# ThomasK33/kube-scheduler-simulator

Hardware: AMD Instinct MI355X
Metric: pod x node filter+score evals/sec (higher is better)
Workload: dtype int64

## Files before the change

### include/ksim_engine.h

```cpp
#ifndef KSIM_ENGINE_H
#define KSIM_ENGINE_H

#include <stdint.h>
#include <stddef.h>

#ifdef __cplusplus
extern "C" {
#endif

#define KSIM_ABI_VERSION 12

#define KSIM_KEY_NODE_MASK    ((1 << 18) - 1)
#define KSIM_MAX_NODES        KSIM_KEY_NODE_MASK
#define KSIM_MAX_NODE_TAINTS  8
#define KSIM_TAINT_WORDS      4
#define KSIM_MAX_SCALAR       8
#define KSIM_MAX_LABEL_COLS   256
#define KSIM_EXPR_VALS        6
#define KSIM_MAX_FILTER       16
#define KSIM_MAX_SCORE        8
#define KSIM_MAX_RES          4
#define KSIM_MAX_SHAPE        16
#define KSIM_MAX_USES         16
#define KSIM_MAX_CLASSES      4096
// ... 264 lines not shown
  int32_t n_feasible;
  int32_t n_evaluated;
  int32_t n_processed;
  int32_t k_to_find;
  int32_t next_start;
  int32_t _pad;
} ksim_eval_out;

typedef struct ksim_batch_stats {
  int64_t pods;
  int64_t scheduled;
  int64_t unschedulable;
  int64_t evals;
  double  device_ms;
  int64_t batches;
  int64_t truncations;
  int64_t perpod_cycles;
} ksim_batch_stats;

typedef struct ksim_handle ksim_handle;

int  ksim_abi_version(void);
size_t ksim_abi_sizeof(int which);
int  ksim_create(int device, ksim_handle** out);
void ksim_destroy(ksim_handle* h);
const char* ksim_last_error(const ksim_handle* h);

int ksim_set_profile(ksim_handle* h, const ksim_profile* p);
int ksim_set_cluster(ksim_handle* h, const ksim_node_table* nodes, const ksim_vocab* vocab);
int ksim_upsert_nodes(ksim_handle* h, const ksim_node_table* nodes, const ksim_vocab* vocab, const int32_t* old_pos);
int ksim_remove_node(ksim_handle* h, int32_t pos);
int ksim_update_node_rows(ksim_handle* h, const ksim_node_table* nodes, const ksim_vocab* vocab, const int32_t* rows,
                          int32_t n_rows);
int ksim_get_node_state(ksim_handle* h, int64_t* req_cpu, int64_t* req_mem, int64_t* req_eph,
                        int64_t* nz_cpu, int64_t* nz_mem, int32_t* num_pods);
int ksim_get_nb_alloc(ksim_handle* h, int64_t* out);
int ksim_get_class_count(ksim_handle* h, int32_t* out);
int ksim_get_next_start(ksim_handle* h, int32_t* next_start);
int ksim_set_next_start(ksim_handle* h, int32_t next_start);
int ksim_set_pod_seq(ksim_handle* h, int64_t seq);

int ksim_eval_pod(ksim_handle* h, const ksim_pod_set* pods, int32_t pod_index, ksim_eval_out* out);

int ksim_eval_pod_filter(ksim_handle* h, const ksim_pod_set* pods, int32_t pod_index, ksim_eval_out* out);
int ksim_eval_pod_finish(ksim_handle* h, const uint8_t* ext_fail, const int64_t* ext_score, ksim_eval_out* out);
int ksim_assume(ksim_handle* h, const ksim_pod_set* pods, int32_t pod_index, int32_t node);
int ksim_forget(ksim_handle* h, const ksim_pod_set* pods, int32_t pod_index, int32_t node);

int ksim_fw_prefilter(ksim_handle* h, const ksim_pod_set* pods, int32_t pod_index, ksim_eval_out* out);
int ksim_fw_score(ksim_handle* h, const int32_t* nodes, int32_t n, ksim_eval_out* out);
int ksim_fw_normalize(ksim_handle* h, int32_t score_slot, const int32_t* nodes, const int64_t* scores, int32_t n,
                      int64_t* out);
int ksim_fw_filter_nominated(ksim_handle* h, const ksim_pod_set* nominated, int32_t n_nodes, const int32_t* nodes,
                             const int32_t* first, const int32_t* count, uint8_t* fail_plugin,
                             uint32_t* fail_detail);

int ksim_load_pods(ksim_handle* h, const ksim_pod_set* pods);
int ksim_schedule_loaded(ksim_handle* h, int32_t first, int32_t count,
                         int32_t* chosen, ksim_batch_stats* stats);
int ksim_schedule_batch(ksim_handle* h, const ksim_pod_set* pods, int32_t* chosen,
                        ksim_batch_stats* stats);

int ksim_reset_cluster(ksim_handle* h);

#define KSIM_SWEEP_MAX_LANES 64
#define KSIM_SWEEP_DEFAULT_LANES 64
int ksim_sweep_loaded(ksim_handle* h, int32_t first, int32_t count, const ksim_profile* profs, int32_t n_profs,
                      int32_t max_lanes, int32_t* chosen ,
                      ksim_batch_stats* stats );

#define KSIM_COMM_ID_BYTES 128
int ksim_set_shard(ksim_handle* h, int32_t node_base, int32_t n_total);
int ksim_set_eval_range(ksim_handle* h, int32_t eval_lo, int32_t eval_hi);
int ksim_comm_unique_id(uint8_t* id );
int ksim_comm_init(ksim_handle* h, int32_t rank, int32_t world, const uint8_t* id);
int ksim_group_schedule_loaded(ksim_handle** hs, int32_t n, int32_t first, int32_t count,
                               int32_t* chosen, ksim_batch_stats* stats);

int ksim_time_kernels(ksim_handle* h, int32_t first, int32_t count, double* avg_ms,
                      int64_t* launches, int32_t cap);
const char* ksim_kernel_name(int32_t k);
int ksim_time_eval(ksim_handle* h, int32_t first, int32_t reps, double* avg_ms, int32_t* kernel);
int ksim_get_diag(ksim_handle* h, int64_t* out, int32_t n);
int ksim_batch_geometry(int32_t* out, int32_t n);

#define KSIM_PREEMPT_REQ (3 + KSIM_MAX_SCALAR)
typedef struct ksim_bound_pods {
  int32_t n, _pad;
  const int32_t* node;
  const int32_t* priority;
  const int64_t* start_time;
  const int64_t* req;
} ksim_bound_pods;

typedef struct ksim_preempt_out {
  int32_t nominated;
  int32_t n_victims;
  int32_t n_potential;
  int32_t n_candidates;
  int32_t* victims;
  int32_t victims_cap;
  int32_t n_pdb_violations;
} ksim_preempt_out;

int ksim_set_bound_pods(ksim_handle* h, const ksim_bound_pods* b);
int ksim_set_bound_pod_adds(ksim_handle* h, const int32_t* off, const ksim_class_add* adds);
int ksim_set_bound_pod_pdbs(ksim_handle* h, int32_t n_pdbs, const int32_t* allowed, const int32_t* off,
                            const int32_t* ids);
int ksim_preempt(ksim_handle* h, const ksim_pod_set* pods, int32_t pod_index, int32_t priority,
                 ksim_preempt_out* out);
int ksim_preempt_nominated(ksim_handle* h, const ksim_pod_set* pods, int32_t pod_index, int32_t priority,
                           const ksim_pod_set* nominated, int32_t n_groups, const int32_t* nodes,
                           const int32_t* first, const int32_t* count, ksim_preempt_out* out);

int ksim_preempt_spread(ksim_handle* h, const ksim_pod_set* pods, int32_t pod_index, int32_t priority,
                        const ksim_pod_set* nominated, int32_t n_groups, const int32_t* nodes,
                        const int32_t* first, const int32_t* count, ksim_preempt_out* out);

typedef struct ksim_match_problem {
  int32_t n_sigs, n_feat, n_reqs, n_matchers;
  const int32_t* sig_feat_off;
  const int32_t* sig_feat;
  const int32_t* req_feat_off;
  const int32_t* req_feat;
  const uint8_t* req_neg;
  const int32_t* m_req_off;
  const int32_t* m_req;
  int32_t n_pods, n_nodes, n_classes, _pad;
  const int32_t* pod_sig;
  const int32_t* pod_node;
  const int32_t* class_matcher;
} ksim_match_problem;

int ksim_match_terms(ksim_handle* h, const ksim_match_problem* mp, uint32_t* match_bits, int32_t* counts);

typedef struct ksim_emit_input {
  int32_t n_nodes, n_filter, n_score, n_messages;
  const char* const* node_names;
  const char* const* filter_names;
  const char* const* score_names;
  const int32_t* score_weight;
  const uint8_t* has_normalize;
  const uint8_t* fail_plugin;
  const int32_t* msg_id;
  const char* const* messages;
  const uint8_t* scored;
  const int64_t* raw;
  const int64_t* norm;
} ksim_emit_input;

int ksim_emit_cycle_json(const ksim_emit_input* in, char* filter_json, int64_t filter_cap, char* score_json,
                         int64_t score_cap, char* final_json, int64_t final_cap, int64_t* lens);

typedef struct ksim_k8s_kv {
  int32_t key, value;
} ksim_k8s_kv;

typedef struct ksim_k8s_taint {
  int32_t key, value, effect;
} ksim_k8s_taint;

typedef struct ksim_k8s_toleration {
  int32_t key, op, value, effect;
} ksim_k8s_toleration;

typedef struct ksim_k8s_requirement {
// ... 186 lines not shown
```

### kube-scheduler-simulator_amd/csrc/ksim_adapt.hip

```cpp
#include "ksim_device.h"
#include "ksim_internal.h"
#include "ksim_wave.h"
#include "ksim_commit.h"
#include "ksim_chain.h"

namespace ksim {

__device__ __forceinline__ bool batch_feasible(const DevCluster& c, const DevPods& P, const BatchProg& bp,
                                               const ksim_pod& p, const NodeRow& r, bool trivial, int32_t pi) {
  if (!trivial) {
    const int32_t scls = P.stab ? P.sclass[pi] : -1;
    if (scls >= 0 ? !stab_pass(P.stab[(size_t)scls * c.n + r.node]) : !static_filters_pass(c, P, bp, p, r))
      return false;
  }
  return !bp.has_fit_filter || !fits_request(r, p, c.n_scalar, c.fit_ignore);
}

__host__ __device__ inline int32_t mask_pods(int32_t n_words) {
  const int32_t wb = (n_words + 3) / 4;
  const int32_t mp = wb / (n_words <= 256 ? 4 : 8);
  return mp < 1 ? 1 : mp > 64 ? 64 : mp;
}

__global__ __launch_bounds__(256) void k_adapt_mask_ns(DevCluster c, DevPods P, const BatchProg* __restrict__ bp_p,
// ... 889 lines not shown
    const uint64_t mm = __ballot(q * 256 + tid < nchain0 && brk[q]);
    if (mm && lane == 0) atomicMin(&s_fb, q * 256 + (tid & ~63) + __builtin_ctzll(mm));
  }
  lds_barrier();
  const int32_t nchain = s_fb;
  if (tid == 0) s_istar = nchain;
  lds_barrier();
#pragma unroll
  for (int q = 0; q < kChunks; q++) {
    const uint64_t mm = __ballot(q * 256 + tid < nchain && m[q] > g[q]);
    if (mm && lane == 0) atomicMin(&s_istar, q * 256 + (tid & ~63) + __builtin_ctzll(mm));
  }
  lds_barrier();
  const int32_t istar = s_istar;
  const int32_t committed = istar < nchain ? istar + 1 : nchain;
#pragma unroll
  for (int q = 0; q < kChunks; q++)
    if (q * 256 + tid == istar && istar < nchain) s_inode = key_node(m[q]) - c.base;
  lds_barrier();
  const int32_t inode = s_inode;
#pragma unroll
  for (int q = 0; q < kChunks; q++) {
    const int32_t t = q * 256 + tid;
    const int32_t gn = (t < istar && g[q]) ? key_node(g[q]) - c.base : -1;
    if (gn >= nbase && gn < nbase + 256) {
      const ksim_pod& pt = P.pods[cur0 + t];
      ResCols d{pt.req_cpu, pt.req_mem, pt.req_eph, pt.nz_cpu, pt.nz_mem, 1};
      if (gn == inode) {
        const ksim_pod& pi = P.pods[cur0 + istar];
        d.cpu += pi.req_cpu;
        d.mem += pi.req_mem;
        d.eph += pi.req_eph;
        d.nzc += pi.nz_cpu;
        d.nzm += pi.nz_mem;
        d.pods += 1;
      }
      s_rq[t] = d;
      s_dn[gn - nbase] = (int16_t)t;
    }
  }
  if (bl == 0) {
#pragma unroll
    for (int q = 0; q < kChunks; q++) {
      const int32_t t = q * 256 + tid;
      if (t < committed) {
        const int32_t pn = t == istar ? inode + c.base : (g[q] ? key_node(g[q]) : -1);
        atomicAdd(pn >= 0 ? &s_sched : &s_unsched, 1);
        const int2 w = reinterpret_cast<const int2*>(w1)[t];
        atomicAdd(&s_evals, (int32_t)window_local(c, w.x, w.y >= 0 ? (int64_t)w.y + 1 : c.n_total));
      }
    }
  }
  if (tid == 0)
    for (int32_t k = bl; k < committed; k += nblocks) {
      const uint64_t gk = L.g1[k];
      if (chosen_out) chosen_out[cur0 + k] = k == istar ? inode + c.base : (gk ? key_node(gk) : -1);
    }
  lds_barrier();
  if (bl == 0 && tid == 0) {
    constexpr int kWords = (int)(sizeof(DevState) / 8);
    uint64_t wd[kWords];
#pragma unroll
    for (int q = 0; q < kWords; q++) wd[q] = reinterpret_cast<const uint64_t*>(L.st_in)[q];
    DevState ns;
    __builtin_memcpy(&ns, wd, sizeof(ns));
    if (e1 > 0) {
      const int32_t nb = min(kBatchPods, end - cur0);
      ns.cursor = cur0 + committed;
      ns.pod_seq = seq0 + committed;
      ns.scheduled += s_sched;
      ns.unschedulable += s_unsched;
      ns.batches += 1;
      ns.cuts += (committed < nb && istar < nchain ? 1 : 0);
      ns.truncations += (committed < nb && istar >= nchain ? 1 : 0);
      if (committed > 0) {
        const int2 w = reinterpret_cast<const int2*>(w1)[committed - 1];
        ns.next_start = (int32_t)(((int64_t)w.x + (w.y >= 0 ? w.y : c.n_total)) % c.n_total);
        if (c.count_whole) ns.evals += s_evals;
      }
    }
    __builtin_memcpy(wd, &ns, sizeof(ns));
#pragma unroll
    for (int q = 0; q < kWords; q++) reinterpret_cast<uint64_t*>(L.st_out)[q] = wd[q];
    if (FLUSH) *L.e_self = -1;
  }
  const int32_t node = nbase + tid;
  const bool on = node < c.n;
  const int32_t x = on ? node : 0;
  const int32_t e = s_dn[tid];
  ResCols d{0, 0, 0, 0, 0, 0};
  if (on && e >= 0) d = s_rq[e];
  const int64_t rc = c.req_cpu[x] + d.cpu, rm = c.req_mem[x] + d.mem, re = c.req_eph[x] + d.eph;
  const int32_t np = c.num_pods[x] + d.pods;
  if (on && blockIdx.y == 0) {
    L.w.req_cpu[x] = rc;
    L.w.req_mem[x] = rm;
    L.w.req_eph[x] = re;
    L.w.nz_cpu[x] = c.nz_cpu[x] + d.nzc;
    L.w.nz_mem[x] = c.nz_mem[x] + d.nzm;
    L.w.num_pods[x] = np;
  }
  if (FLUSH) return;
  const int32_t base = cur0 + committed;
  const int32_t nb = min(kBatchPods, end - base);
  const int32_t j0 = blockIdx.y * mp;
  if (j0 >= nb) return;
  const int32_t w = blockIdx.x * 4 + (tid >> 6);
  if (w >= n_words) return;
  const int32_t j1 = min(j0 + mp, nb);
  const BatchProg& bp = *bp_p;
  const bool fit = bp.has_fit_filter != 0;
  uint64_t word = 0;
  if (!fit) {
    const uint64_t mk = __ballot(on);
    word = lane < j1 - j0 ? mk : 0ull;
  } else {
    __shared__ int64_t s_pq[4][64][4];
    const int wv = tid >> 6;
    if (lane < j1 - j0) {
      const ksim_pod& q = P.pods[base + j0 + lane];
      const bool none = q.req_cpu == 0 && q.req_mem == 0 && q.req_eph == 0 && !(q.flags & KSIM_POD_HAS_SCALAR);
      s_pq[wv][lane][0] = none ? INT64_MIN : q.req_cpu;
      s_pq[wv][lane][1] = none ? INT64_MIN : q.req_mem;
      s_pq[wv][lane][2] = none ? INT64_MIN : q.req_eph;
    }
    const uint64_t room = __ballot(on && np + 1 <= c.alloc_pods[x]);
    const int64_t fc = c.alloc_cpu[x] - rc, fm = c.alloc_mem[x] - rm, fe = c.alloc_eph[x] - re;
    __shared__ uint64_t s_mk[4][64];
#pragma unroll 4
    for (int32_t l = 0; l < j1 - j0; l++) {
      const int64_t c0 = s_pq[wv][l][0], m0 = s_pq[wv][l][1], e0 = s_pq[wv][l][2];
      const uint64_t mk = room & __ballot(c0 <= fc) & __ballot(m0 <= fm) & __ballot(e0 <= fe);
      if (lane == 0) s_mk[wv][l] = mk;
    }
    word = lane < j1 - j0 ? s_mk[wv][lane] : 0ull;
  }
  if (lane < j1 - j0) amask[(size_t)(j0 + lane) * n_words + w] = word;
}

const char* const kAdaptKernelNames[kKernelsPerAdapt] = {"k_adapt_mask", "k_adapt_window", "k_adapt_top",
                                                         "k_adapt_pairs", "k_adapt_commit"};

uint32_t launch_batch_adapt(const LaunchArgs& a, hipStream_t stream, hipEvent_t* evs) {
  const int32_t n_words = (a.c.n + 63) / 64;
  const int32_t k = num_feasible_nodes_to_find(a.prof.percentage_of_nodes_to_score, a.c.n);
  if (evs) (void)hipEventRecord(evs[0], stream);
  const int32_t mp = mask_pods(n_words);
  k_adapt_mask_ns<<<dim3((n_words + 3) / 4, (kBatchPods + mp - 1) / mp), 256, 0, stream>>>(a.c, a.P, a.dbp, a.st,
                                                                                          a.s.amask, n_words, mp);
  if (evs) (void)hipEventRecord(evs[1], stream);
  const bool win_seq = !a.fast && n_words <= kWinSeqWords;
  const bool win_fused = !win_seq && k < kTopWideK && n_words <= kWinFusedWords;
  if (win_seq)
    launch_window_dbl(a, n_words, k, stream);
  else if (!win_fused) {
    k_adapt_cut0<<<kBatchPods / 4, 256, 0, stream>>>(a.st, a.s.amask, n_words, a.c.n, k, a.s.acut);
    k_adapt_window<<<1, kBatchPods, 0, stream>>>(a.st, a.s.amask, n_words, a.c.n, k, a.s.acut, a.s.awin, a.s.aexact);
  }
  if (evs) (void)hipEventRecord(evs[2], stream);
#define TOP(F, NT, W) k_adapt_top<false, F, NT, W><<<kBatchPods, NT, 0, stream>>>(a.c, a.P, a.dprof, a.dbp, a.st, \
    a.s.amask, n_words, a.s.awin, a.s.aexact, a.s.topk, a.s.topk_cnt, a.s.topk_complete, nullptr, a.s.pnorm)
  if (k >= kTopWideK || win_seq) {
    if (a.fast) TOP(true, 1024, false);
    else TOP(false, 1024, false);
  } else if (win_fused) {
    if (a.fast) TOP(true, 256, true);
// ... 121 lines not shown
```

### kube-scheduler-simulator_amd/csrc/ksim_batch.hip

```cpp
#include "ksim_device.h"
#include <atomic>

#include "ksim_internal.h"
#include "ksim_wave.h"
#include "ksim_commit.h"
#include "ksim_chain.h"

namespace ksim {



template <int kTopThreads, int N = kTileCand, bool SORTED = true>
__device__ __forceinline__ void top_finish(uint64_t (&a)[N], int32_t nfeas, int32_t j,
                                           uint64_t* __restrict__ topk, int32_t* __restrict__ topk_cnt,
                                           int32_t* __restrict__ topk_complete, uint64_t* __restrict__ xsend,
                                           uint64_t* tclk = nullptr) {
  constexpr int kTopWaves = kTopThreads / 64;
  constexpr int kTopSlots = (kTopWaves * kTopT + 63) / 64;
  __shared__ uint64_t s_list[kTopWaves][kTopT];
  __shared__ int32_t s_cnt[kTopWaves], s_complete[kTopWaves];
  const int lane = threadIdx.x & 63, wv = threadIdx.x >> 6;
  {
    __shared__ uint64_t s_wmax[kTopWaves], s_wthr[kTopWaves];
    __shared__ int32_t s_wc[kTopWaves], s_wf[kTopWaves];
// ... 815 lines not shown
      d.eph += x.eph;
      d.nzc += x.nzc;
      d.nzm += x.nzm;
      d.pods += 1;
    }
    s_rq[tid] = d;
    if constexpr (RT && !FLUSH) {
      if (twice) {
        const PodReq x = s_pc[committed];
        ksim_pod pq;
        pq.req_cpu = x.cpu;
        pq.req_mem = x.mem;
        pq.req_eph = x.eph;
        pq.nz_cpu = x.nzc;
        pq.nz_mem = x.nzm;
        prow.req_cpu += d.cpu;
        prow.req_mem += d.mem;
        prow.req_eph += d.eph;
        prow.nz_cpu += d.nzc;
        prow.nz_mem += d.nzm;
        prow.num_pods += d.pods;
        pe = req_entry(fast_prog(*bp_p), pq, prow, pic, pim);
      }
      if (live) s_patch[tid] = (uint16_t)pe;
    }
    if constexpr (DIRECT) {
      s_ent[gnode] = (int16_t)tid;
    } else {
      atomicOr(&s_bits[gnode >> 5], 1u << (gnode & 31));
      uint32_t h = lazy_hash(gnode);
      while (atomicCAS(&s_hkey[h], -1, gnode) != -1) h = (h + 1) & (kLazyHash - 1);
      s_hval[h] = (int16_t)tid;
    }
  }
  const int32_t pnode = tid == istar ? inode + c.base : (g1 ? key_node(g1) : -1);
  if (tid == b && tid < committed && chosen_out) chosen_out[cur0 + b] = pnode;
  if (b == 0 && tid < committed) atomicAdd(pnode >= 0 ? &s_sched : &s_unsched, 1);
  int32_t mn0 = -1, mn1 = -1;
  ResCols mr0{0, 0, 0, 0, 0, 0}, mr1{0, 0, 0, 0, 0, 0};
  UpRow ms[RT ? 2 : 1];
  if (tid == b) {
    if (b < nchain && g1) mn0 = key_node(g1) - c.base;
    if (b < e2 && g2) mn1 = key_node(g2) - c.base;
    if (mn0 >= 0) mr0 = ResCols{c.req_cpu[mn0], c.req_mem[mn0], c.req_eph[mn0], c.nz_cpu[mn0], c.nz_mem[mn0], c.num_pods[mn0]};
    if (mn1 >= 0) mr1 = ResCols{c.req_cpu[mn1], c.req_mem[mn1], c.req_eph[mn1], c.nz_cpu[mn1], c.nz_mem[mn1], c.num_pods[mn1]};
    if constexpr (RT) {
      const int32_t mn[2] = {mn0, mn1};
#pragma unroll
      for (int w = 0; w < 2; w++) {
        const int32_t n = mn[w] >= 0 ? mn[w] : 0;
        ms[w].alloc_cpu = c.alloc_cpu[n];
        ms[w].alloc_mem = c.alloc_mem[n];
        ms[w].alloc_eph = c.alloc_eph[n];
        ms[w].inv_cpu = c.inv_cpu[n];
        ms[w].inv_mem = c.inv_mem[n];
        ms[w].alloc_pods = c.alloc_pods[n];
        ms[w].node = mn[w];
      }
    }
  }
  lds_barrier();
  auto update_state = [&]() {
    static_assert(sizeof(DevState) % 8 == 0, "DevState by words");
    constexpr int kWords = (int)(sizeof(DevState) / 8);
    uint64_t w[kWords];
#pragma unroll
    for (int q = 0; q < kWords; q++) w[q] = reinterpret_cast<const uint64_t*>(L.st_in)[q];
    DevState ns;
    __builtin_memcpy(&ns, w, sizeof(ns));
    if (e1 > 0) {
      const int32_t nb = min(kBatchPods, end - cur0);
      ns.cursor = base;
      ns.pod_seq = seq0 + committed;
      ns.scheduled += s_sched;
      ns.unschedulable += s_unsched;
      ns.batches += 1;
      ns.cuts += (committed < nb && istar < nchain ? 1 : 0);
      ns.truncations += (committed < nb && istar >= nchain ? 1 : 0);
      ns.evals += (int64_t)committed * (c.eval_hi - c.eval_lo);
    }
    __builtin_memcpy(w, &ns, sizeof(ns));
#pragma unroll
    for (int q = 0; q < kWords; q++) reinterpret_cast<uint64_t*>(L.st_out)[q] = w[q];
    if (FLUSH) *L.e_self = -1;
  };
  const bool st_writer = b == 0 && tid == kThreads - 64;
  auto delta = [&](int32_t node) -> ResCols {
    if constexpr (DIRECT) {
      return s_rq[s_ent[node]];
    } else {
      ResCols d{0, 0, 0, 0, 0, 0};
      const uint32_t bw = s_bits[node >> 5], bit = 1u << (node & 31);
      if (bw & bit) {
        uint32_t h = lazy_hash(node);
        while (s_hkey[h] != node) h = (h + 1) & (kLazyHash - 1);
        d = s_rq[s_hval[h]];
      }
      return d;
    }
  };
  auto write_row = [&](int32_t mn, const ResCols& mr, int which) {
    ResCols s = mr;
    if (mn >= 0) {
      const ResCols d = delta(mn);
      s = ResCols{mr.cpu + d.cpu, mr.mem + d.mem, mr.eph + d.eph, mr.nzc + d.nzc, mr.nzm + d.nzm, mr.pods + d.pods};
      L.w.req_cpu[mn] = s.cpu;
      L.w.req_mem[mn] = s.mem;
      L.w.req_eph[mn] = s.eph;
      L.w.nz_cpu[mn] = s.nzc;
      L.w.nz_mem[mn] = s.nzm;
      L.w.num_pods[mn] = s.pods;
    }
    if constexpr (RT) {
      ms[which].s = s;
      s_up[which] = ms[which];
    }
  };
  auto materialize = [&]() {
    if (tid != b) return;
    write_row(mn0, mr0, 0);
    write_row(mn1, mr1, 1);
  };
  auto upkeep = [&]() {
    if constexpr (RT) {
      const int32_t t = tid - 64;
      if (t < 0 || t >= 2 * rt.n_cls) return;
      const UpRow& u = s_up[t < rt.n_cls ? 0 : 1];
      const int32_t mn = u.node;
      if (mn < 0) return;
      NodeRow r;
      r.alloc_cpu = u.alloc_cpu;
      r.alloc_mem = u.alloc_mem;
      r.alloc_eph = u.alloc_eph;
      r.alloc_pods = u.alloc_pods;
      r.req_cpu = u.s.cpu;
      r.req_mem = u.s.mem;
      r.req_eph = u.s.eph;
      r.nz_cpu = u.s.nzc;
      r.nz_mem = u.s.nzm;
      r.num_pods = u.s.pods;
      ksim_pod pq;
      pq.req_cpu = creq.cpu;
      pq.req_mem = creq.mem;
      pq.req_eph = creq.eph;
      pq.nz_cpu = creq.nzc;
      pq.nz_mem = creq.nzm;
      const int32_t k = t < rt.n_cls ? t : t - rt.n_cls;
      rt.t_out[(size_t)k * (size_t)c.n + mn] = (uint16_t)req_entry(fast_prog(*bp_p), pq, r, u.inv_cpu, u.inv_mem);
    }
  };
  if (!live) {
    materialize();
    if constexpr (RT) {
      lds_barrier();
      upkeep();
    }
    if (st_writer) update_state();
    return;
  }
  if constexpr (NS) {
    const int32_t s = b % kNsSlices;
    const int32_t len = c.eval_hi - c.eval_lo, S = (len + kNsSlices - 1) / kNsSlices;
    const int32_t slo = c.eval_lo + s * S, shi = min(c.eval_hi, slo + S);
    const FastProg bq = fast_prog(*bp_p);
    const int32_t cu = __builtin_amdgcn_readfirstlane(committed);
    ksim_pod pf[kNsPods];
// ... 433 lines not shown
```

### kube-scheduler-simulator_amd/csrc/ksim_engine.cpp

```cpp
#include <dlfcn.h>
#include <hip/hip_runtime.h>
#include <rccl/rccl.h>

#include <algorithm>
#include <array>
#include <cstdio>
#include <cstdlib>
#include <cstring>
#include <map>
#include <string>
#include <tuple>
#include <unordered_map>
#include <type_traits>
#include <vector>

#include "ksim_internal.h"

using namespace ksim;

namespace {

constexpr int kGraphCycles = 128;

struct Rccl {
  bool ok = false;
  decltype(&ncclGetUniqueId) get_unique_id = nullptr;
  decltype(&ncclCommInitRank) comm_init_rank = nullptr;
  decltype(&ncclCommDestroy) comm_destroy = nullptr;
  decltype(&ncclAllGather) all_gather = nullptr;
  decltype(&ncclAllReduce) all_reduce = nullptr;
  decltype(&ncclGetErrorString) error_string = nullptr;
};

const Rccl& rccl() {
  static Rccl r = [] {
    Rccl x;
    void* lib = nullptr;
    for (const char* name : {"librccl.so", "librccl.so.1"})
      if (!lib) lib = dlopen(name, RTLD_NOW | RTLD_NOLOAD);
    for (const char* name : {"librccl.so.1", "librccl.so", "/opt/rocm/lib/librccl.so.1"})
      if (!lib) lib = dlopen(name, RTLD_NOW | RTLD_GLOBAL);
    if (!lib) return x;
    x.get_unique_id = (decltype(x.get_unique_id))dlsym(lib, "ncclGetUniqueId");
    x.comm_init_rank = (decltype(x.comm_init_rank))dlsym(lib, "ncclCommInitRank");
    x.comm_destroy = (decltype(x.comm_destroy))dlsym(lib, "ncclCommDestroy");
    x.all_gather = (decltype(x.all_gather))dlsym(lib, "ncclAllGather");
    x.all_reduce = (decltype(x.all_reduce))dlsym(lib, "ncclAllReduce");
    x.error_string = (decltype(x.error_string))dlsym(lib, "ncclGetErrorString");
    x.ok = x.get_unique_id && x.comm_init_rank && x.comm_destroy && x.all_gather && x.all_reduce && x.error_string;
    return x;
  }();
  return r;
}
constexpr int kGraphBatches = 16;

struct DevBuf {
  void* p = nullptr;
  size_t bytes = 0;
};

struct DevArena {
  void* p = nullptr;
  size_t cap = 0;
};

}

struct PodBlob {
  std::vector<char> bytes;
  size_t off[8];
  int32_t n_nn, n_exprs, n_terms, n_uses, n_adds;
};

struct ksim_handle {
  int device = 0;
  hipStream_t stream = nullptr;
  hipEvent_t ev0 = nullptr, ev1 = nullptr;
  std::string err;

  bool has_profile = false;
  ksim_profile prof{};
  BatchProg bp{};
  ksim_profile* d_prof = nullptr;
  BatchProg* d_bp = nullptr;
  std::vector<size_t> pod_buf_bytes;

  bool has_cluster = false;
  DevCluster dc{};
// ... 59 lines not shown
  size_t pin_cap = 0;
  struct PinSlot {
    void* p = nullptr;
    void* d = nullptr;
    size_t cap = 0;
    hipEvent_t ev = nullptr;
    bool pending = false;
  };
  static constexpr int kPinRing = 4;
  PinSlot ring[kPinRing];
  int ring_next = 0;
  std::vector<char> pod1_blob;
  char* pod1_base = nullptr;
  std::vector<ksim_label_expr> bs_ex;
  std::vector<ksim_term> bs_tm;
  std::vector<ksim_topo_use> bs_us;
  std::vector<ksim_class_add> bs_ad;
  std::vector<int32_t> bs_nn;
  PodBlob fw_blob;
  DevArena fw_arena[2];
  int fw_flip = 0;
  struct PendBind {
    bool on = false;
    DevPods P{};
    int32_t node = 0;
    int sign = 0;
  } pend_bind;
  int64_t pend_reuse = 0;
  void* pout = nullptr;
  void* pout_d = nullptr;
  size_t pout_cap = 0;
  std::vector<DevBuf> pre_bufs;
  std::vector<DevBuf> pre_nom_bufs;
  int64_t* pre_smin = nullptr;
  std::vector<DevBuf> pre_add_bufs;
  std::vector<DevBuf> pre_pdb_bufs;
  DevPreempt pre{};
  std::vector<int32_t> pre_index;
  int32_t pre_n = 0;
  DevPods pod1{};
  bool ext_pending = false;
  uint8_t* ext_fail = nullptr;
  int64_t* ext_score = nullptr;
  bool fw_pending = false, fw_scored = false, fw_dom_dirty = false, fw_topo = false;
  int32_t fw_ns = 0;
  std::vector<uint8_t> fw_fail;
  std::vector<int32_t> fw_list;
  std::vector<int64_t> fw_raw, fw_norm;
  bool fw_host = false;
  int64_t fw_counts[4] = {0, 0, 0, 0};
  std::vector<uint8_t> fw_seen;
  std::vector<int64_t> fw_tot;
  void* fwh = nullptr;
  void* fwh_d = nullptr;
  size_t fwh_cap = 0;
  uint32_t fw_tflags = 0;
  size_t fw_oraw = 0, fw_opart = 0;
  bool fw_raw32 = false;
  int32_t* fw_nodes = nullptr;
  int64_t* fw_vals = nullptr;
  int64_t* fw_out = nullptr;

  int32_t shard_base = 0, shard_total = 0;
  bool replicated = false;
  int32_t eval_lo = 0, eval_hi = 0;
  bool rep_primary = true;
  int32_t rank = 0, world = 1;
  ncclComm_t comm = nullptr;

  hipGraphExec_t graph_cycle[16] = {};
  hipGraphExec_t graph_batch = nullptr;
  hipGraphExec_t graph_batch_fast = nullptr;
  hipGraphExec_t graph_batch_stab = nullptr;
  hipGraphExec_t graph_tbatch = nullptr;
  std::vector<DevBuf> lazy_bufs;
  int32_t lazy_n = -1;
  DynCols lazy_x1{};
  DevState* lazy_st1 = nullptr;
  uint64_t *lazy_g = nullptr, *lazy_m = nullptr;
  int32_t* lazy_e = nullptr;
  int32_t *lazy_ab = nullptr, *lazy_aw = nullptr;
  hipGraphExec_t graph_lazy = nullptr;
  hipGraphExec_t graph_lazy_adapt = nullptr;
  std::vector<uint16_t> rq_cls;
  uint16_t* d_rcls = nullptr;
  PodReq* d_rreq = nullptr;
  int32_t rq_ncls = 0;
  std::vector<DevBuf> rtab_bufs;
  size_t rtab_bytes = 0;
  hipGraphExec_t graph_lazy_rt = nullptr;
  int64_t rtab_runs = 0;
  int32_t rt_graph_ncls = 0;
  std::vector<DevBuf> ash_bufs;
  uint64_t *ash_send = nullptr, *ash_recv = nullptr, *ash_gmask = nullptr;
  int32_t ash_world = 0, ash_w = 0;
  struct SweepLaneBufs {
    DynCols x[2];
    uint64_t *g, *m;
    int32_t* e;
    uint64_t* topk;
    int32_t *topk_cnt, *topk_complete, *pinv;
    int64_t* pnorm;
  };
  void* sweep_slab = nullptr;
  int32_t sweep_n = -1, sweep_lanes = 0;
  std::vector<SweepLaneBufs> sweep_lane;
  DevState* sweep_st = nullptr;
  SweepLane* sweep_tab = nullptr;
  DevArena sweep_profs, sweep_rows;
  std::map<std::pair<int32_t, bool>, hipGraphExec_t> sweep_graphs;
  int64_t graph_captures = 0;
  int64_t graph_gen = 0;
  std::vector<std::pair<const ksim_handle*, int64_t>> sg_sig;
  std::map<std::tuple<bool, int64_t, int64_t>, hipGraphExec_t> sg_graphs;
  bool sg_off = false;
  int64_t match_ns = 0;
};

namespace {

int set_err(ksim_handle* h, int code, const std::string& msg) {
  if (h) h->err = msg;
  return code;
}

int hip_fail(ksim_handle* h, hipError_t e, const char* what) {
  int code = (e == hipErrorOutOfMemory) ? KSIM_E_OOM : KSIM_E_DEVICE;
  return set_err(h, code, std::string(what) + ": " + hipGetErrorString(e));
}

#define HIPCHK(h, expr)                                    \
  do {                                                     \
    hipError_t _e = (expr);                                \
    if (_e != hipSuccess) return hip_fail((h), _e, #expr); \
  } while (0)

static hipError_t hcopy(ksim_handle* h, void* dst, const void* src, size_t bytes, hipMemcpyKind kind) {
  const hipError_t e = hipMemcpyAsync(dst, src, bytes, kind, h->stream);
  return e != hipSuccess ? e : hipStreamSynchronize(h->stream);
}

static hipError_t hzero(ksim_handle* h, void* dst, size_t bytes) {
  const hipError_t e = hipMemsetAsync(dst, 0, bytes, h->stream);
  return e != hipSuccess ? e : hipStreamSynchronize(h->stream);
}

void free_bufs(std::vector<DevBuf>& v) {
  for (auto& b : v)
    if (b.p) (void)hipFree(b.p);
  v.clear();
}

int upload(ksim_handle* h, std::vector<DevBuf>& owner, const void* src, size_t bytes, void** out) {
  void* p = nullptr;
  size_t alloc = bytes ? bytes : 16;
  hipError_t e = hipMalloc(&p, alloc);
  if (e != hipSuccess) return hip_fail(h, e, "hipMalloc");
  owner.push_back({p, alloc});
  if (src && bytes) {
    e = hipMemcpyAsync(p, src, bytes, hipMemcpyHostToDevice, h->stream);
  } else {
    e = hipMemsetAsync(p, 0, alloc, h->stream);
  }
  if (e != hipSuccess) return hip_fail(h, e, "upload copy");
  *out = p;
  return KSIM_OK;
}

void drop_cycle_graphs(ksim_handle* h) {
  for (auto& g : h->graph_cycle) {
    if (g) (void)hipGraphExecDestroy(g);
    g = nullptr;
  }
  for (auto& kv : h->sg_graphs) (void)hipGraphExecDestroy(kv.second);
  h->sg_graphs.clear();
  h->graph_gen++;
}

void drop_graphs(ksim_handle* h) {
  drop_cycle_graphs(h);
  for (auto& kv : h->sweep_graphs)
    if (kv.second) (void)hipGraphExecDestroy(kv.second);
  h->sweep_graphs.clear();
  if (h->graph_batch) (void)hipGraphExecDestroy(h->graph_batch);
  if (h->graph_batch_fast) (void)hipGraphExecDestroy(h->graph_batch_fast);
  if (h->graph_batch_stab) (void)hipGraphExecDestroy(h->graph_batch_stab);
  h->graph_batch_stab = nullptr;
  if (h->graph_tbatch) (void)hipGraphExecDestroy(h->graph_tbatch);
  if (h->graph_lazy) (void)hipGraphExecDestroy(h->graph_lazy);
  if (h->graph_lazy_adapt) (void)hipGraphExecDestroy(h->graph_lazy_adapt);
  h->graph_lazy_adapt = nullptr;
  if (h->graph_lazy_rt) (void)hipGraphExecDestroy(h->graph_lazy_rt);
  h->graph_lazy_rt = nullptr;
  h->graph_batch_fast = nullptr;
  h->graph_batch = nullptr;
  h->graph_tbatch = nullptr;
  h->graph_lazy = nullptr;
}

bool plugin_supported(int id) { return id >= 0 && id < KSIM_PL_COUNT; }
bool is_sharded(const ksim_handle* h);

int validate_pod(ksim_handle* h, const ksim_pod_set* ps, int32_t i) {
  const ksim_pod& p = ps->pods[i];
  const DevCluster& c = h->dc;
  if (p.flags & (KSIM_POD_HAS_HOST_PORTS | KSIM_POD_HAS_VOLUMES))
    return set_err(h, KSIM_E_UNSUPPORTED, "pod " + std::to_string(i) + ": host ports / volumes not supported by the engine");
  if (p.node_name < -2 || p.node_name >= c.n_total)
    return set_err(h, KSIM_E_INVALID, "pod " + std::to_string(i) + ": node_name out of range");
  auto check_expr = [&](int32_t e) -> bool {
    if (e < 0 || e >= ps->n_exprs) return false;
    const ksim_label_expr& x = ps->exprs[e];
    if (x.nvals > KSIM_EXPR_VALS || x.op > KSIM_OP_TRUE) return false;
    if (x.op <= KSIM_OP_LT && x.col >= c.n_label_cols) return false;
    return true;
  };
  auto check_terms = [&](int32_t first, int32_t count) -> bool {
    if (count < 0 || (count > 0 && (first < 0 || first + count > ps->n_terms))) return false;
    for (int32_t t = 0; t < count; t++) {
      const ksim_term& tm = ps->terms[first + t];
      if (tm.n_expr < 0) return false;
      for (int32_t k = 0; k < tm.n_expr; k++)
        if (!check_expr(tm.first_expr + k)) return false;
    }
    return true;
  };
  if (p.sel_count < 0) return set_err(h, KSIM_E_INVALID, "bad sel_count");
  for (int32_t k = 0; k < p.sel_count; k++)
    if (!check_expr(p.sel_first + k)) return set_err(h, KSIM_E_INVALID, "pod " + std::to_string(i) + ": bad nodeSelector expr");
  if (!check_terms(p.req_term_first, p.req_term_count) || !check_terms(p.pref_term_first, p.pref_term_count))
    return set_err(h, KSIM_E_INVALID, "pod " + std::to_string(i) + ": bad affinity term range");
  if ((p.flags & KSIM_POD_ADDED_AFFINITY) && (p.added_term_count <= 0 || !check_terms(p.added_term_first, p.added_term_count)))
    return set_err(h, KSIM_E_INVALID, "pod " + std::to_string(i) + ": bad addedAffinity term range");
  const std::string who = "pod " + std::to_string(i) + ": ";
  for (const auto& vl : {std::make_pair(p.vb_first, p.vb_count), std::make_pair(p.vz_first, p.vz_count)}) {
    if (vl.second == 0) continue;
    if (!check_terms(vl.first, vl.second)) return set_err(h, KSIM_E_INVALID, who + "bad volume term range");
    for (int32_t k = 0; k < vl.second; k++) {
      const int32_t g = ps->terms[vl.first + k].weight;
      if (g < 0 || (k > 0 && g < ps->terms[vl.first + k - 1].weight))
        return set_err(h, KSIM_E_INVALID, who + "volume term groups must be non-decreasing");
    }
  }
  if (p.use_count < 0 || p.use_count > KSIM_MAX_USES ||
      (p.use_count > 0 && (!ps->uses || p.use_first < 0 || p.use_first + p.use_count > ps->n_uses)))
    return set_err(h, KSIM_E_INVALID, who + "bad topology use range");
  for (int32_t k = 0; k < p.use_count; k++) {
    const ksim_topo_use& u = ps->uses[p.use_first + k];
    if (u.kind > KSIM_USE_IMAGE) return set_err(h, KSIM_E_INVALID, who + "bad topology use kind");
    if (u.cls < -1 || u.cls >= c.n_classes) return set_err(h, KSIM_E_INVALID, who + "topology use class out of range");
    if (u.col != KSIM_COL_NONE && u.col >= c.n_label_cols)
      return set_err(h, KSIM_E_INVALID, who + "topology key column out of range");
    if (u.kind == KSIM_USE_PTS_SOFT && c.n_topo_log < c.n + 1)
      return set_err(h, KSIM_E_INVALID, who + "ScheduleAnyway spread needs topo_log[0..n_nodes]");
  }
  if (p.add_count < 0 || (p.add_count > 0 && (!ps->adds || p.add_first < 0 || p.add_first + p.add_count > ps->n_adds)))
    return set_err(h, KSIM_E_INVALID, who + "bad class add range");
  for (int32_t k = 0; k < p.add_count; k++)
    if (ps->adds[p.add_first + k].cls < 0 || ps->adds[p.add_first + k].cls >= c.n_classes)
      return set_err(h, KSIM_E_INVALID, who + "class add out of range");
  if (p.flags & KSIM_POD_NODE_NAMES) {
    if (p.nn_count < 0 || (p.nn_count > 0 && (!ps->nn || p.nn_first < 0 ||
                                              (int64_t)p.nn_first + p.nn_count > (int64_t)ps->n_nn)))
      return set_err(h, KSIM_E_INVALID, who + "bad PreFilterResult node range");
    for (int32_t k = 0; k < p.nn_count; k++) {
      const int32_t v = ps->nn[p.nn_first + k];
      if (v < 0 || v >= c.n_total || (k > 0 && v <= ps->nn[p.nn_first + k - 1]))
        return set_err(h, KSIM_E_INVALID, who + "PreFilterResult nodes must be increasing node positions");
    }
    if (is_sharded(h))
      return set_err(h, KSIM_E_UNSUPPORTED, who + "a PreFilterResult node restriction runs on unsharded handles");
  }
  return KSIM_OK;
}

bool static_trivial(const ksim_handle* h, const ksim_pod& p) {
  if (p.node_name != -1 || p.sel_count > 0 || (p.flags & (KSIM_POD_HAS_REQUIRED_AFFINITY | KSIM_POD_ADDED_AFFINITY)))
    return false;
  if (h->any_unschedulable && !(p.flags & KSIM_POD_TOLERATES_UNSCHEDULABLE)) return false;
  for (uint16_t id : h->hard_taints)
// ... 251 lines not shown
int capture(ksim_handle* h, bool batch, bool topo, hipGraphExec_t* out, bool fast = false, bool fuse_min = false,
            bool fuse_ext = false, bool ptab = false, bool stab = false) {
  HIPCHK(h, hipStreamSynchronize(h->stream));
  LaunchArgs a = make_args(h, h->dp, h->d_chosen);
  a.fast = fast;
  a.stab = stab;
  a.fuse_min = fuse_min;
  a.fuse_ext = fuse_ext;
  a.ptab = ptab;
  hipGraph_t g = nullptr;
  HIPCHK(h, hipStreamBeginCapture(h->stream, hipStreamCaptureModeThreadLocal));
  if (batch)
    for (int i = 0; i < kGraphBatches; i++) {
      if (adapt_mode(h))
        launch_batch_adapt(a, h->stream);
      else
        launch_batch(a, h->stream);
    }
  else
    for (int i = 0; i < kGraphCycles; i++) launch_cycle(a, h->stream, false, topo);
  hipError_t e = hipStreamEndCapture(h->stream, &g);
  if (e != hipSuccess) return hip_fail(h, e, "hipStreamEndCapture");
  e = hipGraphInstantiate(out, g, nullptr, nullptr, 0);
  (void)hipGraphDestroy(g);
  if (e != hipSuccess) return hip_fail(h, e, "hipGraphInstantiate");
  h->graph_captures++;
  return KSIM_OK;
}


int run_tbatch(ksim_handle* h, int32_t a, int32_t b, const LaunchArgs& la) {
  int rc;
  HIPCHK(h, hipMemsetAsync(h->sc.tb_win, 0, sizeof(WinState) * kTbPods, h->stream));
  HIPCHK(h, hipMemsetAsync(h->sc.tb_dom, 0, sizeof(TbDom) * kTbPods * kVarDom, h->stream));
  HIPCHK(h, hipMemsetAsync(h->sc.tb_vhold, 0, 4 * (size_t)kTbPods * kVarSlots * 2 * KSIM_MAX_SCORE, h->stream));
  if (!h->graph_tbatch) {
    HIPCHK(h, hipStreamSynchronize(h->stream));
    hipGraph_t g = nullptr;
    HIPCHK(h, hipStreamBeginCapture(h->stream, hipStreamCaptureModeThreadLocal));
    for (int i = 0; i < kGraphBatches; i++) launch_tbatch(la, h->stream);
    hipError_t e = hipStreamEndCapture(h->stream, &g);
    if (e != hipSuccess) return hip_fail(h, e, "hipStreamEndCapture");
    e = hipGraphInstantiate(&h->graph_tbatch, g, nullptr, nullptr, 0);
    (void)hipGraphDestroy(g);
    if (e != hipSuccess) {
      h->graph_tbatch = nullptr;
      return hip_fail(h, e, "hipGraphInstantiate");
    }
    h->graph_captures++;
  }
  int32_t cursor = a;
  while (cursor < b) {
    int32_t nbat = 0;
    for (int32_t i = cursor; i < b; nbat++) i += std::min(std::min(kTbPods, b - i), std::max(h->tlen[i], 1));
    int32_t done = 0;
    for (; done + kGraphBatches <= nbat; done += kGraphBatches) HIPCHK(h, hipGraphLaunch(h->graph_tbatch, h->stream));
    for (; done < nbat; done++) launch_tbatch(la, h->stream);
    HIPCHK(h, hipGetLastError());
    DevState st;
    if ((rc = read_state(h, st))) return rc;
    if (st.cursor <= cursor) return set_err(h, KSIM_E_DEVICE, "topology batch path made no progress");
    cursor = st.cursor;
  }
  return KSIM_OK;
}

bool lazy_enabled() {
  constexpr bool off = ab(kAbLazy);
  return !off;
}

bool lazy_ok(const ksim_handle* h, int32_t a, int32_t b, bool fast, bool stab = false) {
  if (!lazy_enabled() || !fast || stab) return false;
  if (adapt_mode(h) ? (is_sharded(h) && !h->replicated) : (is_sharded(h) || h->replicated)) return false;
  if (h->dc.base != 0 || h->dc.n > kLazyMaxNodes || h->dc.n <= 0) return false;
  for (int32_t i = a; i < b; i++)
    if (!h->noadd[i]) return false;
  return true;
}

int alloc_lazy(ksim_handle* h) {
  if (h->lazy_n == h->dc.n) return KSIM_OK;
  HIPCHK(h, hipStreamSynchronize(h->stream));
  if (h->graph_lazy) (void)hipGraphExecDestroy(h->graph_lazy);
  if (h->graph_lazy_adapt) (void)hipGraphExecDestroy(h->graph_lazy_adapt);
  if (h->graph_lazy_rt) (void)hipGraphExecDestroy(h->graph_lazy_rt);
  h->graph_lazy = h->graph_lazy_adapt = h->graph_lazy_rt = nullptr;
  free_bufs(h->lazy_bufs);
  h->lazy_n = -1;
  const size_t n = (size_t)h->dc.n;
  int rc;
  void* p = nullptr;
  int64_t** cols[5] = {&h->lazy_x1.req_cpu, &h->lazy_x1.req_mem, &h->lazy_x1.req_eph, &h->lazy_x1.nz_cpu,
                       &h->lazy_x1.nz_mem};
  for (auto* c : cols) {
    if ((rc = upload(h, h->lazy_bufs, nullptr, 8 * n, &p))) return rc;
    *c = (int64_t*)p;
  }
  if ((rc = upload(h, h->lazy_bufs, nullptr, 4 * n, &p))) return rc;
  h->lazy_x1.num_pods = (int32_t*)p;
  if ((rc = upload(h, h->lazy_bufs, nullptr, sizeof(DevState), &p))) return rc;
  h->lazy_st1 = (DevState*)p;
  if ((rc = upload(h, h->lazy_bufs, nullptr, 8 * (size_t)kLazySlots * kBatchPods, &p))) return rc;
  h->lazy_g = (uint64_t*)p;
  if ((rc = upload(h, h->lazy_bufs, nullptr, 8 * (size_t)kLazySlots * kBatchPods, &p))) return rc;
  h->lazy_m = (uint64_t*)p;
  if ((rc = upload(h, h->lazy_bufs, nullptr, 4 * (size_t)kLazySlots, &p))) return rc;
  h->lazy_e = (int32_t*)p;
  if ((rc = upload(h, h->lazy_bufs, nullptr, 4 * (size_t)kLazySlots * kBatchPods, &p))) return rc;
  h->lazy_ab = (int32_t*)p;
  if ((rc = upload(h, h->lazy_bufs, nullptr, 8 * (size_t)kLazySlots * kBatchPods, &p))) return rc;
  h->lazy_aw = (int32_t*)p;
  h->lazy_n = h->dc.n;
  return KSIM_OK;
}

DynCols dyn_cols(const DevCluster& c) {
  return DynCols{c.req_cpu, c.req_mem, c.req_eph, c.nz_cpu, c.nz_mem, c.num_pods};
}

DevCluster with_cols(DevCluster c, const DynCols& d) {
  c.req_cpu = d.req_cpu;
  c.req_mem = d.req_mem;
  c.req_eph = d.req_eph;
  c.nz_cpu = d.nz_cpu;
  c.nz_mem = d.nz_mem;
  c.num_pods = d.num_pods;
  return c;
}

bool reqtab_enabled() {
  constexpr bool off = ab(kAbReqTab);
  return !off;
}

bool reqtab_ok(const ksim_handle* h, int32_t a, int32_t b) {
  if (!reqtab_enabled() || adapt_mode(h) || !fast_def(h->bp)) return false;
  if (h->dc.n > kKeepPerLane * 1024) return false;
  const int32_t C = h->rq_ncls;
  if (C <= 0 || C > kReqMaxClasses || (int64_t)(b - a) < 8 * (int64_t)C || !h->d_rcls) return false;
  for (int32_t i = a; i < b; i++)
    if (h->rq_cls[(size_t)i] == 0xffff) return false;
  return true;
}

size_t rtab_halves_bytes(const ksim_handle* h) {
  const size_t t = 2 * sizeof(uint16_t) * (size_t)h->rq_ncls * (size_t)h->dc.n;
  return (t + 255) & ~(size_t)255;
}
int ensure_rtab(ksim_handle* h) {
  const size_t need = rtab_halves_bytes(h) + sizeof(uint16_t) * kLazySlots * (size_t)h->rq_ncls * kBatchPods;
  if (h->rtab_bytes >= need && !h->rtab_bufs.empty()) return KSIM_OK;
  HIPCHK(h, hipStreamSynchronize(h->stream));
  if (h->graph_lazy_rt) (void)hipGraphExecDestroy(h->graph_lazy_rt);
  h->graph_lazy_rt = nullptr;
  free_bufs(h->rtab_bufs);
  h->rtab_bytes = 0;
  void* p = nullptr;
  int rc;
  if ((rc = upload(h, h->rtab_bufs, nullptr, need, &p))) return rc;
  h->rtab_bytes = need;
  return KSIM_OK;
}

LazyBatch lazy_batch(const ksim_handle* h, const LaunchArgs& la, int64_t i, bool rt = false) {
  const int p = (int)(i & 1), q = (int)(i & 3), q1 = (int)((i + 3) & 3), q2 = (int)((i + 2) & 3);
  const DynCols x[2] = {dyn_cols(h->dc), h->lazy_x1};
  DevState* st[2] = {h->st, h->lazy_st1};
  LazyBatch z;
  z.a = la;
  z.a.c = with_cols(la.c, x[p ^ 1]);
  z.cw = with_cols(la.c, x[p]);
  z.step.w = x[p];
  z.step.st_in = st[p ^ 1];
  z.step.st_out = st[p];
  z.step.g1 = h->lazy_g + (size_t)q1 * kBatchPods;
  z.step.m1 = h->lazy_m + (size_t)q1 * kBatchPods;
  z.step.e1 = h->lazy_e + q1;
  z.step.g2 = h->lazy_g + (size_t)q2 * kBatchPods;
  z.step.e2 = h->lazy_e + q2;
  z.step.e_self = h->lazy_e + q;
  z.st = st[p];
  z.gkey = h->lazy_g + (size_t)q * kBatchPods;
  z.pmax = h->lazy_m + (size_t)q * kBatchPods;
  z.cend = h->lazy_e + q;
  z.b1 = h->lazy_ab + (size_t)q1 * kBatchPods;
  z.w1 = h->lazy_aw + (size_t)q1 * 2 * kBatchPods;
  z.abroken = h->lazy_ab + (size_t)q * kBatchPods;
  z.awin = h->lazy_aw + (size_t)q * 2 * kBatchPods;
  if (rt) {
    uint16_t* const t = (uint16_t*)h->rtab_bufs[0].p;
    const size_t half = (size_t)h->rq_ncls * (size_t)h->dc.n;
    z.rt.t_in = t + (size_t)(p ^ 1) * half;
    z.rt.t_out = t + (size_t)p * half;
    z.rt.rreq = h->d_rreq;
    z.rt.rcls = h->d_rcls;
    z.rt.n_cls = h->rq_ncls;
    uint16_t* const pe = (uint16_t*)((char*)h->rtab_bufs[0].p + rtab_halves_bytes(h));
    const size_t slot = (size_t)h->rq_ncls * kBatchPods;
    z.rt.p_in = pe + (size_t)q1 * slot;
    z.rt.p_out = pe + (size_t)q * slot;
  }
  return z;
}

int lazy_begin(ksim_handle* h) {
  int rc;
  if ((rc = alloc_lazy(h))) return rc;
  const size_t n = (size_t)h->dc.n;
  const DynCols x0 = dyn_cols(h->dc), x1 = h->lazy_x1;
  HIPCHK(h, hipMemcpyAsync(x1.req_cpu, x0.req_cpu, 8 * n, hipMemcpyDeviceToDevice, h->stream));
  HIPCHK(h, hipMemcpyAsync(x1.req_mem, x0.req_mem, 8 * n, hipMemcpyDeviceToDevice, h->stream));
  HIPCHK(h, hipMemcpyAsync(x1.req_eph, x0.req_eph, 8 * n, hipMemcpyDeviceToDevice, h->stream));
  HIPCHK(h, hipMemcpyAsync(x1.nz_cpu, x0.nz_cpu, 8 * n, hipMemcpyDeviceToDevice, h->stream));
  HIPCHK(h, hipMemcpyAsync(x1.nz_mem, x0.nz_mem, 8 * n, hipMemcpyDeviceToDevice, h->stream));
  HIPCHK(h, hipMemcpyAsync(x1.num_pods, x0.num_pods, 4 * n, hipMemcpyDeviceToDevice, h->stream));
  HIPCHK(h, hipMemcpyAsync(h->lazy_st1, h->st, sizeof(DevState), hipMemcpyDeviceToDevice, h->stream));
  HIPCHK(h, hipMemsetAsync(h->lazy_e, 0xff, 4 * kLazySlots, h->stream));
  return KSIM_OK;
}

int lazy_end(ksim_handle* h, int64_t f) {
  if ((f & 1) == 0) return KSIM_OK;
  const size_t n = (size_t)h->dc.n;
  const DynCols x0 = dyn_cols(h->dc), x1 = h->lazy_x1;
  HIPCHK(h, hipMemcpyAsync(x0.req_cpu, x1.req_cpu, 8 * n, hipMemcpyDeviceToDevice, h->stream));
  HIPCHK(h, hipMemcpyAsync(x0.req_mem, x1.req_mem, 8 * n, hipMemcpyDeviceToDevice, h->stream));
  HIPCHK(h, hipMemcpyAsync(x0.req_eph, x1.req_eph, 8 * n, hipMemcpyDeviceToDevice, h->stream));
  HIPCHK(h, hipMemcpyAsync(x0.nz_cpu, x1.nz_cpu, 8 * n, hipMemcpyDeviceToDevice, h->stream));
  HIPCHK(h, hipMemcpyAsync(x0.nz_mem, x1.nz_mem, 8 * n, hipMemcpyDeviceToDevice, h->stream));
  HIPCHK(h, hipMemcpyAsync(x0.num_pods, x1.num_pods, 4 * n, hipMemcpyDeviceToDevice, h->stream));
  HIPCHK(h, hipMemcpyAsync(h->st, h->lazy_st1, sizeof(DevState), hipMemcpyDeviceToDevice, h->stream));
  return KSIM_OK;
}

int read_state_at(ksim_handle* h, const DevState* src, DevState& st) {
  HIPCHK(h, hipMemcpyAsync(&st, src, sizeof(st), hipMemcpyDeviceToHost, h->stream));
  HIPCHK(h, hipStreamSynchronize(h->stream));
  return KSIM_OK;
}

uint32_t lazy_launch(const ksim_handle* h, const LazyBatch& z, hipStream_t stream, hipEvent_t* evs = nullptr) {
  return adapt_mode(h) ? launch_batch_adapt_lazy(z, stream, evs) : launch_batch_lazy(z, stream, evs);
}

void lazy_flush(const ksim_handle* h, const LazyBatch& z, hipStream_t stream) {
  if (adapt_mode(h)) launch_adapt_lazy_flush(z, stream);
  else launch_lazy_flush(z, stream);
}

int reqtab_begin(ksim_handle* h, const LaunchArgs& la) {
  int rc;
  if ((rc = ensure_rtab(h))) return rc;
  const LazyBatch z0 = lazy_batch(h, la, 0, true);
  launch_req_table(la, z0.rt, z0.rt.t_out, const_cast<uint16_t*>(z0.rt.t_in), h->stream);
  return KSIM_OK;
}

int run_lazy(ksim_handle* h, int32_t a, int32_t b, const LaunchArgs& la) {
  int rc;
  if ((rc = lazy_begin(h))) return rc;
  const bool rt = reqtab_ok(h, a, b);
  if (rt) {
    h->rtab_runs++;
    if ((rc = reqtab_begin(h, la))) return rc;
  }
  if (rt && h->graph_lazy_rt && h->rt_graph_ncls != h->rq_ncls) {
    HIPCHK(h, hipStreamSynchronize(h->stream));
    (void)hipGraphExecDestroy(h->graph_lazy_rt);
    h->graph_lazy_rt = nullptr;
  }
  hipGraphExec_t& graph = adapt_mode(h) ? h->graph_lazy_adapt : rt ? h->graph_lazy_rt : h->graph_lazy;
  if (!graph) {
    if (rt) h->rt_graph_ncls = h->rq_ncls;
    HIPCHK(h, hipStreamSynchronize(h->stream));
    hipGraph_t g = nullptr;
    HIPCHK(h, hipStreamBeginCapture(h->stream, hipStreamCaptureModeThreadLocal));
    for (int i = 0; i < kGraphBatches; i++) lazy_launch(h, lazy_batch(h, la, i, rt), h->stream);
    hipError_t e = hipStreamEndCapture(h->stream, &g);
    if (e != hipSuccess) return hip_fail(h, e, "hipStreamEndCapture");
    e = hipGraphInstantiate(&graph, g, nullptr, nullptr, 0);
    (void)hipGraphDestroy(g);
    if (e != hipSuccess) {
      graph = nullptr;
      return hip_fail(h, e, "hipGraphInstantiate");
    }
    h->graph_captures++;
  }
  static_assert(kGraphBatches % kLazySlots == 0, "lazy graphs keep the ring phase");
  int64_t i = 0;
  int32_t cursor = a;
  while (cursor < b) {
    int32_t nb = (b - cursor + kBatchPods - 1) / kBatchPods;
    const int32_t align = (int32_t)((kLazySlots - (i & 3)) & 3);
    if (nb >= align + kGraphBatches) {
      for (int32_t r = 0; r < align; r++, i++, nb--) lazy_launch(h, lazy_batch(h, la, i, rt), h->stream);
      for (int32_t r = 0; r < nb / kGraphBatches; r++, i += kGraphBatches) HIPCHK(h, hipGraphLaunch(graph, h->stream));
    } else {
      for (int32_t r = 0; r < nb; r++, i++) lazy_launch(h, lazy_batch(h, la, i, rt), h->stream);
    }
    lazy_flush(h, lazy_batch(h, la, i, rt), h->stream);
    HIPCHK(h, hipGetLastError());
    DevState st;
    if ((rc = read_state_at(h, (i & 1) ? h->lazy_st1 : h->st, st))) return rc;
    if (st.cursor <= cursor) return set_err(h, KSIM_E_DEVICE, "deferred-commit batch path made no progress");
    cursor = st.cursor;
    i++;
  }
  return lazy_end(h, i - 1);
}

int alloc_sweep(ksim_handle* h, int32_t lanes) {
  if (!h->sweep_tab) {
    void* t = nullptr;
    hipError_t e = hipMalloc(&t, sizeof(SweepLane) * kLazySlots * kSweepMaxLanes);
    if (e != hipSuccess) return hip_fail(h, e, "hipMalloc");
    h->sweep_tab = (SweepLane*)t;
  }
  if (h->sweep_n == h->dc.n && lanes <= h->sweep_lanes) return KSIM_OK;
  HIPCHK(h, hipStreamSynchronize(h->stream));
  if (h->sweep_slab) (void)hipFree(h->sweep_slab);
  h->sweep_slab = nullptr;
  h->sweep_n = -1;
  h->sweep_lanes = 0;
  h->sweep_lane.clear();
  const size_t n = (size_t)h->dc.n;
  size_t off = 0;
  auto take = [&](size_t bytes) {
    const size_t at = off;
    off += (bytes + 255) & ~(size_t)255;
    return at;
  };
  struct Off {
    size_t col[2][6], g, m, e, topk, cnt, cmp, pnorm, pinv;
  };
  std::vector<Off> offs((size_t)lanes);
  const size_t st_off = take(sizeof(DevState) * 2 * (size_t)lanes);
  for (auto& o : offs) {
    for (int p = 0; p < 2; p++)
      for (int k = 0; k < 6; k++) o.col[p][k] = take(k < 5 ? 8 * n : 4 * n);
    o.g = take(8 * (size_t)kLazySlots * kBatchPods);
    o.m = take(8 * (size_t)kLazySlots * kBatchPods);
    o.e = take(4 * (size_t)kLazySlots);
    o.topk = take(8 * (size_t)kBatchPods * kTopT);
    o.cnt = take(4 * (size_t)kBatchPods);
    o.cmp = take(4 * (size_t)kBatchPods);
    o.pnorm = take(8 * (size_t)kBatchPods * 4);
    o.pinv = take(4 * (size_t)kBatchPods);
  }
  void* slab = nullptr;
  hipError_t e = hipMalloc(&slab, off);
  if (e != hipSuccess) return hip_fail(h, e, "hipMalloc");
  if ((e = hipMemsetAsync(slab, 0, off, h->stream)) != hipSuccess) {
    (void)hipFree(slab);
    return hip_fail(h, e, "hipMemsetAsync");
  }
  char* base = (char*)slab;
  h->sweep_slab = slab;
  h->sweep_st = (DevState*)(base + st_off);
  for (const auto& o : offs) {
    ksim_handle::SweepLaneBufs b{};
    for (int p = 0; p < 2; p++)
      b.x[p] = DynCols{(int64_t*)(base + o.col[p][0]), (int64_t*)(base + o.col[p][1]), (int64_t*)(base + o.col[p][2]),
                       (int64_t*)(base + o.col[p][3]), (int64_t*)(base + o.col[p][4]), (int32_t*)(base + o.col[p][5])};
    b.g = (uint64_t*)(base + o.g);
    b.m = (uint64_t*)(base + o.m);
    b.e = (int32_t*)(base + o.e);
    b.topk = (uint64_t*)(base + o.topk);
    b.topk_cnt = (int32_t*)(base + o.cnt);
    b.topk_complete = (int32_t*)(base + o.cmp);
    b.pnorm = (int64_t*)(base + o.pnorm);
    b.pinv = (int32_t*)(base + o.pinv);
    h->sweep_lane.push_back(b);
  }
  h->sweep_n = h->dc.n;
  h->sweep_lanes = lanes;
  return KSIM_OK;
}

int sweep_reserve(ksim_handle* h, DevArena& a, size_t bytes) {
  if (a.cap >= bytes && a.p) return KSIM_OK;
  HIPCHK(h, hipStreamSynchronize(h->stream));
  if (a.p) (void)hipFree(a.p);
  a.p = nullptr;
  a.cap = 0;
  const hipError_t e = hipMalloc(&a.p, bytes ? bytes : 16);
  if (e != hipSuccess) {
    a.p = nullptr;
    return hip_fail(h, e, "hipMalloc");
  }
  a.cap = bytes ? bytes : 16;
  return KSIM_OK;
// ... 68 lines not shown
      htab[(size_t)q * kSweepMaxLanes + l] =
          sweep_record(h, l, q, rows + (size_t)l * np, d_profs + std::max(v, 0), d_bps + std::max(v, 0));
    vec[(size_t)l] = v;
    cur[(size_t)l] = a;
    return KSIM_OK;
  };
  for (int32_t l = 0; l < lanes; l++) {
    const int32_t v = next_v < n_profs ? next_v++ : -1;
    if ((rc = arm(l, v))) return rc;
    live += v >= 0;
  }
  HIPCHK(h, hipMemcpyAsync(tab, htab.data(), sizeof(SweepLane) * htab.size(), hipMemcpyHostToDevice, h->stream));
  hipGraphExec_t& graph = h->sweep_graphs[{lanes, def}];
  if (!graph && count >= kBatchPods * kGraphBatches) {
    HIPCHK(h, hipStreamSynchronize(h->stream));
    hipGraph_t g = nullptr;
    HIPCHK(h, hipStreamBeginCapture(h->stream, hipStreamCaptureModeThreadLocal));
    for (int i = 0; i < kGraphBatches; i++)
      launch_sweep_batch(c, P, tab + (size_t)(i & 3) * kSweepMaxLanes, lanes, def, h->stream);
    hipError_t e = hipStreamEndCapture(h->stream, &g);
    if (e != hipSuccess) return hip_fail(h, e, "hipStreamEndCapture");
    e = hipGraphInstantiate(&graph, g, nullptr, nullptr, 0);
    (void)hipGraphDestroy(g);
    if (e != hipSuccess) {
      graph = nullptr;
      return hip_fail(h, e, "hipGraphInstantiate");
    }
    h->graph_captures++;
  }
  auto phase_tab = [&](int64_t i) { return tab + (size_t)(i & 3) * kSweepMaxLanes; };
  int64_t i = 0;
  while (live > 0) {
    int32_t nb = 0;
    for (int32_t l = 0; l < lanes; l++)
      if (vec[(size_t)l] >= 0) nb = std::max(nb, (b - cur[(size_t)l] + kBatchPods - 1) / kBatchPods);
    const int32_t align = (int32_t)((kLazySlots - (i & 3)) & 3);
    nb = std::min(nb, align + kGraphBatches);
    if (graph && nb >= align + kGraphBatches) {
      for (int32_t r = 0; r < align; r++, i++, nb--) launch_sweep_batch(c, P, phase_tab(i), lanes, def, h->stream);
      for (int32_t r = 0; r < nb / kGraphBatches; r++, i += kGraphBatches) HIPCHK(h, hipGraphLaunch(graph, h->stream));
    } else {
      for (int32_t r = 0; r < nb; r++, i++) launch_sweep_batch(c, P, phase_tab(i), lanes, def, h->stream);
    }
    launch_sweep_flush(c, P, phase_tab(i), lanes, h->stream);
    HIPCHK(h, hipGetLastError());
    HIPCHK(h, hipMemcpyAsync(hst.data(), h->sweep_st, sizeof(DevState) * hst.size(), hipMemcpyDeviceToHost, h->stream));
    HIPCHK(h, hipStreamSynchronize(h->stream));
    bool progress = false, retab = false;
    for (int32_t l = 0; l < lanes; l++) {
      const int32_t v = vec[(size_t)l];
      if (v < 0) continue;
      const DevState& st = hst[2 * (size_t)l + (size_t)(i & 1)];
      progress = progress || st.cursor > cur[(size_t)l];
      cur[(size_t)l] = st.cursor;
      if (st.cursor < b) continue;
      if (count)
        HIPCHK(h, hipMemcpyAsync(chosen + (size_t)v * count, rows + (size_t)l * np + a, 4 * (size_t)count,
                                 hipMemcpyDeviceToHost, h->stream));
      if (stats) {
        ksim_batch_stats& o = stats[v];
        o.pods = count;
        o.scheduled = st.scheduled;
        o.unschedulable = st.unschedulable;
        o.evals = st.evals;
        o.device_ms = 0;
        o.batches = st.batches;
        o.truncations = st.truncations;
        o.perpod_cycles = 0;
      }
      const int32_t nv = next_v < n_profs ? next_v++ : -1;
      if ((rc = arm(l, nv))) return rc;
      live -= nv < 0;
      retab = true;
    }
    if (!progress) return set_err(h, KSIM_E_DEVICE, "packed sweep made no progress");
    if (retab)
      HIPCHK(h, hipMemcpyAsync(tab, htab.data(), sizeof(SweepLane) * htab.size(), hipMemcpyHostToDevice, h->stream));
    i++;
  }
  HIPCHK(h, hipStreamSynchronize(h->stream));
  return KSIM_OK;
}

int run_range(ksim_handle* h, int32_t a, int32_t b, bool batch, bool topo) {
  int rc;
  if ((rc = set_run(h, a, b))) return rc;
  LaunchArgs la = make_args(h, h->dp, h->d_chosen);
  if (!batch) {
    la.fuse_min = topo;
    for (int32_t i = a; i < b && la.fuse_min; i++) la.fuse_min = h->hard_small[i] != 0;
    la.fuse_ext = true;
    for (int32_t i = a; i < b && la.fuse_ext; i++) la.fuse_ext = h->soft_le1[i] != 0;
    la.ptab = h->topo[a] == 2;
    hipGraphExec_t& g =
        h->graph_cycle[(topo ? 1 : 0) | (la.fuse_min ? 2 : 0) | (la.fuse_ext ? 4 : 0) | (la.ptab ? 8 : 0)];
    if (!g && (rc = capture(h, false, topo, &g, false, la.fuse_min, la.fuse_ext, la.ptab))) return rc;
    int32_t done = a;
    for (; done + kGraphCycles <= b; done += kGraphCycles) HIPCHK(h, hipGraphLaunch(g, h->stream));
    for (; done < b; done++) launch_cycle(la, h->stream, false, topo);
    HIPCHK(h, hipGetLastError());
    return KSIM_OK;
  }
  if (topo) return run_tbatch(h, a, b, la);
  pick_keys(h, a, b, la);
  if (lazy_ok(h, a, b, la.fast, la.stab)) return run_lazy(h, a, b, la);
  hipGraphExec_t& gb = la.stab ? h->graph_batch_stab : la.fast ? h->graph_batch_fast : h->graph_batch;
  if (!gb && (rc = capture(h, true, false, &gb, la.fast, false, false, false, la.stab))) return rc;
  int32_t cursor = a;
  while (cursor < b) {
    const int32_t left = b - cursor;
    if (left >= kBatchPods * kGraphBatches) {
      const int reps = left / (kBatchPods * kGraphBatches);
      for (int r = 0; r < reps; r++) HIPCHK(h, hipGraphLaunch(gb, h->stream));
    } else {
      const int n1 = (left + kBatchPods - 1) / kBatchPods;
      for (int r = 0; r < n1; r++) {
        if (adapt_mode(h))
          launch_batch_adapt(la, h->stream);
        else
          launch_batch(la, h->stream);
      }
      HIPCHK(h, hipGetLastError());
    }
    DevState st;
    if ((rc = read_state(h, st))) return rc;
    if (st.cursor <= cursor) return set_err(h, KSIM_E_DEVICE, "batch path made no progress");
    cursor = st.cursor;
  }
  return KSIM_OK;
}

template <typename F>
int for_each_run(ksim_handle* h, int32_t first, int32_t count, F&& fn, bool adapt_sharded = false) {
  int32_t i = first;
  const int32_t end = first + count;
  while (i < end) {
    const bool batch_ok = !(adapt_mode(h) && is_sharded(h)) || adapt_sharded;
    const bool b = batch_ok && pod_on_batch(h, i);
    const bool t = h->topo[i] != 0;
    int32_t j = i + 1;
    while (j < end && (batch_ok && pod_on_batch(h, j)) == b && h->topo[j] == h->topo[i]) j++;
    int rc = fn(i, j, b, t);
    if (rc) return rc;
    i = j;
  }
  return KSIM_OK;
}

LaunchArgs shard_args(ksim_handle* h, bool fast) {
  LaunchArgs la = make_args(h, h->dp, h->d_chosen);
  la.fast = fast;
  if (h->replicated) {
    la.c.eval_lo = h->eval_lo;
    la.c.eval_hi = h->eval_hi;
  }
  return la;
}

int shard_batch(const std::vector<ksim_handle*>& hs, hipStream_t stream, bool fast) {
  const int R = (int)hs.size();
  ksim_handle* h0 = hs[0];
  const size_t rec = (size_t)kBatchPods * kXRec;
  for (auto* h : hs) launch_shard_eval(shard_args(h, fast), stream);
  if (h0->comm) {
    const ncclResult_t r = rccl().all_gather(h0->sc.xsend, h0->sc.xrecv, rec, ncclUint64, h0->comm, stream);
    if (r != ncclSuccess) return set_err(h0, KSIM_E_RCCL, std::string("ncclAllGather: ") + rccl().error_string(r));
  } else {
    for (int src = 0; src < R; src++)
      for (int dst = 0; dst < R; dst++)
        HIPCHK(h0, hipMemcpyAsync(hs[dst]->sc.xrecv + (size_t)src * rec, hs[src]->sc.xsend, 8 * rec,
                                  hipMemcpyDeviceToDevice, stream));
  }
  const int32_t world = h0->comm ? h0->world : R;
  for (auto* h : hs) launch_shard_chain(shard_args(h, fast), world, stream);
  if (h0->replicated) {
  } else if (h0->comm) {
    const ncclResult_t r =
        rccl().all_reduce(h0->sc.pmax, h0->sc.pmax, kBatchPods, ncclUint64, ncclMax, h0->comm, stream);
    if (r != ncclSuccess) return set_err(h0, KSIM_E_RCCL, std::string("ncclAllReduce: ") + rccl().error_string(r));
  } else if (R > 1) {
    GroupPtrs g{};
    g.n = R;
    for (int i = 0; i < R; i++) g.p[i] = hs[i]->sc.pmax;
    launch_group_max(g, stream);
  }
  for (auto* h : hs) launch_shard_commit(shard_args(h, fast), stream);
  HIPCHK(h0, hipGetLastError());
  return KSIM_OK;
// ... 508 lines not shown

size_t ksim_abi_sizeof(int which) {
  switch (which) {
    case 0: return sizeof(ksim_node_table);
    case 1: return sizeof(ksim_vocab);
    case 2: return sizeof(ksim_label_expr);
    case 3: return sizeof(ksim_term);
    case 4: return sizeof(ksim_pod);
    case 5: return sizeof(ksim_pod_set);
    case 6: return sizeof(ksim_profile);
    case 7: return sizeof(ksim_eval_out);
    case 8: return sizeof(ksim_batch_stats);
    case 9: return sizeof(ksim_topo_use);
    case 10: return sizeof(ksim_class_add);
    case 11: return sizeof(ksim_match_problem);
    case 12: return sizeof(ksim_k8s_kv);
    case 13: return sizeof(ksim_k8s_taint);
    case 14: return sizeof(ksim_k8s_toleration);
    case 15: return sizeof(ksim_k8s_requirement);
    case 16: return sizeof(ksim_k8s_selector_term);
    case 17: return sizeof(ksim_k8s_preferred_term);
    case 18: return sizeof(ksim_k8s_label_selector);
    case 19: return sizeof(ksim_k8s_pod_term);
    case 20: return sizeof(ksim_k8s_spread);
    case 21: return sizeof(ksim_k8s_port);
    case 22: return sizeof(ksim_k8s_container);
    case 23: return sizeof(ksim_k8s_image);
    case 24: return sizeof(ksim_k8s_volume_group);
    case 25: return sizeof(ksim_k8s_node);
    case 26: return sizeof(ksim_k8s_pod);
    case 27: return sizeof(ksim_k8s_namespace);
    case 28: return sizeof(ksim_k8s_service);
    case 29: return sizeof(ksim_k8s_controller);
    case 30: return sizeof(ksim_k8s_pool);
    case 31: return sizeof(ksim_encode_nodes_opts);
    case 32: return sizeof(ksim_encode_pods_opts);
    case 33: return sizeof(ksim_encoder_info);
    default: return 0;
  }
}

int ksim_create(int device, ksim_handle** out) {
  if (!out) return KSIM_E_INVALID;
  *out = nullptr;
  int ndev = 0;
  if (hipGetDeviceCount(&ndev) != hipSuccess || ndev <= 0) return KSIM_E_DEVICE;
  if (device < 0 || device >= ndev) return KSIM_E_INVALID;
  auto* h = new ksim_handle();
  h->device = device;
  if (hipSetDevice(device) != hipSuccess || hipStreamCreateWithFlags(&h->stream, hipStreamNonBlocking) != hipSuccess ||
      hipEventCreate(&h->ev0) != hipSuccess || hipEventCreate(&h->ev1) != hipSuccess ||
      hipMalloc(&h->st, sizeof(DevState)) != hipSuccess || hipMemset(h->st, 0, sizeof(DevState)) != hipSuccess ||
      hipMalloc(&h->d_prof, sizeof(ksim_profile)) != hipSuccess ||
      hipMalloc(&h->d_bp, sizeof(BatchProg)) != hipSuccess) {
    delete h;
    return KSIM_E_DEVICE;
  }
  *out = h;
  return KSIM_OK;
}

void ksim_destroy(ksim_handle* h) {
  if (!h) return;
  (void)hipSetDevice(h->device);
  if (h->stream) (void)hipStreamSynchronize(h->stream);
  drop_graphs(h);
  if (h->comm && rccl().ok) (void)rccl().comm_destroy(h->comm);
  free_bufs(h->cluster_bufs);
  free_bufs(h->scratch_bufs);
  free_bufs(h->ash_bufs);
  free_bufs(h->lazy_bufs);
  if (h->sweep_slab) (void)hipFree(h->sweep_slab);
  if (h->sweep_tab) (void)hipFree(h->sweep_tab);
  if (h->sweep_profs.p) (void)hipFree(h->sweep_profs.p);
  if (h->sweep_rows.p) (void)hipFree(h->sweep_rows.p);
  free_bufs(h->stab_bufs);
  free_bufs(h->rtab_bufs);
  free_bufs(h->pod_bufs);
  if (h->pod1_arena.p) (void)hipFree(h->pod1_arena.p);
  if (h->nom_arena.p) (void)hipFree(h->nom_arena.p);
  for (auto& a : h->fw_arena)
    if (a.p) (void)hipFree(a.p);
  if (h->fwh) (void)hipHostFree(h->fwh);
  if (h->pin) (void)hipHostFree(h->pin);
  if (h->pout) (void)hipHostFree(h->pout);
  free_bufs(h->pre_bufs);
  free_bufs(h->pre_nom_bufs);
  free_bufs(h->pre_add_bufs);
  free_bufs(h->pre_pdb_bufs);
  if (h->d_chosen) (void)hipFree(h->d_chosen);
  if (h->st) (void)hipFree(h->st);
  if (h->d_prof) (void)hipFree(h->d_prof);
  if (h->d_bp) (void)hipFree(h->d_bp);
  for (auto& r : h->ring) {
    if (r.p) (void)hipHostFree(r.p);
    if (r.ev) (void)hipEventDestroy(r.ev);
  }
  if (h->ev0) (void)hipEventDestroy(h->ev0);
  if (h->ev1) (void)hipEventDestroy(h->ev1);
  if (h->stream) (void)hipStreamDestroy(h->stream);
  delete h;
}

const char* ksim_last_error(const ksim_handle* h) { return h ? h->err.c_str() : "null handle"; }

static int validate_profile(ksim_handle* h, const ksim_profile* p) {
  if (p->n_filter < 0 || p->n_filter > KSIM_MAX_FILTER || p->n_score < 0 || p->n_score > KSIM_MAX_SCORE)
    return set_err(h, KSIM_E_INVALID, "plugin count out of range");
  for (int i = 0; i < p->n_filter; i++) {
    if (!plugin_supported(p->filter[i])) return set_err(h, KSIM_E_INVALID, "unknown filter plugin id");
    for (int j = 0; j < i; j++)
      if (p->filter[j] == p->filter[i]) return set_err(h, KSIM_E_INVALID, "filter plugin listed twice");
  }
  for (int i = 0; i < p->n_score; i++) {
    if (!plugin_supported(p->score[i])) return set_err(h, KSIM_E_INVALID, "unknown score plugin id");
    for (int j = 0; j < i; j++)
      if (p->score[j] == p->score[i]) return set_err(h, KSIM_E_INVALID, "score plugin listed twice");
    if (p->score_weight[i] < 0) return set_err(h, KSIM_E_INVALID, "negative score weight");
  }
  if (p->fit_n_res < 0 || p->fit_n_res > KSIM_MAX_RES || p->ba_n_res < 0 || p->ba_n_res > KSIM_MAX_RES)
    return set_err(h, KSIM_E_INVALID, "scoring resources out of range");
  if (p->fit_strategy < KSIM_FIT_LEAST_ALLOCATED || p->fit_strategy > KSIM_FIT_REQUESTED_TO_CAPACITY_RATIO)
    return set_err(h, KSIM_E_INVALID, "unknown NodeResourcesFit scoring strategy");
  if (p->fit_strategy == KSIM_FIT_REQUESTED_TO_CAPACITY_RATIO) {
    if (p->fit_n_shape < 1 || p->fit_n_shape > KSIM_MAX_SHAPE)
      return set_err(h, KSIM_E_INVALID, "RequestedToCapacityRatio shape: 1..16 points");
    for (int i = 0; i < p->fit_n_shape; i++) {
      if (p->fit_shape_util[i] < 0 || p->fit_shape_util[i] > 100 || (i > 0 && p->fit_shape_util[i] <= p->fit_shape_util[i - 1]))
        return set_err(h, KSIM_E_INVALID, "RequestedToCapacityRatio shape: utilization strictly increasing in [0, 100]");
      if (p->fit_shape_score[i] < 0 || p->fit_shape_score[i] > 100 || p->fit_shape_score[i] % 10 != 0)
        return set_err(h, KSIM_E_INVALID, "RequestedToCapacityRatio shape: score x 10 in [0, 100]");
    }
  }
  if (p->fit_ignored_scalar >> KSIM_MAX_SCALAR) return set_err(h, KSIM_E_INVALID, "fit_ignored_scalar past the scalar columns");
  if (p->preempt_min_pct < 0 || p->preempt_min_pct > 100 || p->preempt_min_abs < 0 ||
      (p->preempt_min_pct == 0 && p->preempt_min_abs == 0))
    return set_err(h, KSIM_E_INVALID, "DefaultPreemptionArgs: minCandidateNodesPercentage in [0, 100], "
                                      "minCandidateNodesAbsolute >= 0, not both 0");
  return KSIM_OK;
}

static BatchProg compile_batch_prog(const ksim_profile* p) {
  BatchProg bp{};
  bp.cpu_mem = p->fit_strategy == KSIM_FIT_LEAST_ALLOCATED && p->fit_n_res == 2 && p->fit_res[0] == KSIM_RES_CPU &&
               p->fit_res[1] == KSIM_RES_MEMORY && p->ba_n_res == 2 && p->ba_res[0] == KSIM_RES_CPU &&
               p->ba_res[1] == KSIM_RES_MEMORY;
  bp.fit_w_cpu = p->fit_res_weight[0];
  bp.fit_w_mem = p->fit_res_weight[1];
  bp.fast_w = bp.cpu_mem && bp.fit_w_cpu >= 1 && bp.fit_w_cpu < (1ll << 31) && bp.fit_w_mem >= 1 &&
              bp.fit_w_mem < (1ll << 31);
  bp.no_score = p->n_score == 0;
  bp.fit_w_eq = bp.fast_w && bp.fit_w_cpu == bp.fit_w_mem;
  if (bp.fast_w) {
    bp.inv_w[0] = 1.0 / (double)bp.fit_w_cpu;
    bp.inv_w[1] = 1.0 / (double)bp.fit_w_mem;
    bp.inv_w[2] = 1.0 / (double)(bp.fit_w_cpu + bp.fit_w_mem);
  }
  for (int i = 0; i < p->n_filter; i++) {
    const int f = p->filter[i];
    if (f == KSIM_PL_NODE_UNSCHEDULABLE || f == KSIM_PL_NODE_NAME || f == KSIM_PL_TAINT_TOLERATION ||
        f == KSIM_PL_NODE_AFFINITY)
      bp.static_filter[bp.n_static++] = (uint8_t)f;
    if (f == KSIM_PL_NODE_RESOURCES_FIT) bp.has_fit_filter = 1;
  }
  for (int k = 0; k < p->n_score; k++) {
    const int64_t w = p->score_weight[k] == 0 ? 1 : p->score_weight[k];
// ... 1794 lines not shown
             (tcross[(size_t)i] ? kPodTbCross : 0);
    plans[i].flags |= (uint32_t)(tvcol[(size_t)i] + 1) << kPlanVcolShift;
  }
  DevPods P{};
  void* p = nullptr;
  if ((rc = put(ps->pods, sizeof(ksim_pod) * ps->n_pods, &p))) return drop_queue(rc);
  P.pods = (const ksim_pod*)p;
  if ((rc = put(ps->exprs, sizeof(ksim_label_expr) * ps->n_exprs, &p))) return drop_queue(rc);
  P.exprs = (const ksim_label_expr*)p;
  if ((rc = put(ps->terms, sizeof(ksim_term) * ps->n_terms, &p))) return drop_queue(rc);
  P.terms = (const ksim_term*)p;
  if ((rc = put(ps->nn, 4 * (size_t)ps->n_nn, &p))) return drop_queue(rc);
  P.nn = (const int32_t*)p;
  if ((rc = put(bf.data(), 4 * bf.size(), &p))) return drop_queue(rc);
  P.bflags = (const int32_t*)p;
  if ((rc = put(uses.data(), sizeof(ksim_topo_use) * uses.size(), &p))) return drop_queue(rc);
  P.uses = (const ksim_topo_use*)p;
  if ((rc = put(plans.data(), sizeof(PodPlan) * plans.size(), &p))) return drop_queue(rc);
  P.plans = (const PodPlan*)p;
  if ((rc = put(ps->adds, sizeof(ksim_class_add) * (size_t)ps->n_adds, &p))) return drop_queue(rc);
  P.adds = (const ksim_class_add*)p;
  if ((rc = put(scls.data(), 4 * np1, &p))) return drop_queue(rc);
  h->d_sclass = (int32_t*)p;
  if ((rc = put(srep.data(), 4 * np1, &p))) return drop_queue(rc);
  h->d_srep = (int32_t*)p;
  h->stab_ncls = ncls;
  h->sclass.assign(scls.begin(), scls.begin() + ps->n_pods);
  h->stab_dirty = true;
  h->d_rcls = nullptr;
  h->rq_ncls = 0;
  if ((rc = put(rcls.data(), 2 * np1, &p))) return drop_queue(rc);
  uint16_t* const d_rcls = (uint16_t*)p;
  if ((rc = put(rreq.data(), sizeof(PodReq) * rreq.size(), &p))) return drop_queue(rc);
  h->d_rreq = (PodReq*)p;
  h->d_rcls = d_rcls;
  h->rq_cls.assign(rcls.begin(), rcls.begin() + ps->n_pods);
  h->rq_ncls = n_rcls;
  if ((rc = put(R.ent.data(), sizeof(int4) * R.ent.size(), &p))) return drop_queue(rc);
  P.ptab_ent = (const int4*)p;
  if ((rc = put(R.cfirst.data(), 4 * R.cfirst.size(), &p))) return drop_queue(rc);
  P.ptab_cfirst = R.cfirst.empty() ? nullptr : (const int32_t*)p;
  if ((rc = put(R.cidx.data(), 4 * R.cidx.size(), &p))) return drop_queue(rc);
  P.ptab_cidx = (const int32_t*)p;
  if ((rc = put(nullptr, 8 * (size_t)R.len, &p))) return drop_queue(rc);
  P.ptab = (int64_t*)p;
  P.n_ptab = (int32_t)R.ent.size();
  if ((rc = put(R.padd.data(), sizeof(int4) * R.padd.size(), &p))) return drop_queue(rc);
  P.ptab_padd = (const int4*)p;
  P.n_uses = ps->n_uses;
  P.n_adds = ps->n_adds;
  P.n_nn = ps->n_nn;
  P.n_pods = ps->n_pods;
  P.n_exprs = ps->n_exprs;
  P.n_terms = ps->n_terms;
  hipError_t e = hipSuccess;
  if (!reuse) {
    e = hipMalloc(&h->d_chosen, 4 * np1);
    if (e != hipSuccess) {
      h->d_chosen = nullptr;
      return drop_queue(hip_fail(h, e, "hipMalloc"));
    }
    h->pod_buf_bytes = bytes;
  }
  if ((e = hipMemsetAsync(h->d_chosen, 0xff, 4 * np1, h->stream)) != hipSuccess ||
      (e = hipStreamSynchronize(h->stream)) != hipSuccess)
    return drop_queue(hip_fail(h, e, "pod queue setup"));
  h->batchable = std::move(batchable);
  h->dp = P;
  launch_ptab_init(h->dc, P, h->stream);
  if ((e = hipGetLastError()) != hipSuccess || (e = hipStreamSynchronize(h->stream)) != hipSuccess) {
    h->dp = DevPods{};
    return drop_queue(hip_fail(h, e, "persistent tables"));
  }
  return KSIM_OK;
}

int ksim_schedule_loaded(ksim_handle* h, int32_t first, int32_t count, int32_t* chosen, ksim_batch_stats* stats) {
  int rc = ensure_ready(h);
  if (rc) return rc;
  if (!h->dp.pods && count > 0) return set_err(h, KSIM_E_INVALID, "no pods loaded");
  if (first < 0 || count < 0 || first + count > h->dp.n_pods) return set_err(h, KSIM_E_INVALID, "range out of loaded pods");
  HIPCHK(h, hipSetDevice(h->device));
  if ((rc = ensure_stab(h))) return rc;
  if ((rc = reset_counters(h, h->stream))) return rc;
  int64_t perpod = 0;
  HIPCHK(h, hipEventRecord(h->ev0, h->stream));
  if (is_sharded(h)) {
    for (int32_t i = first; i < first + count; i++) perpod += pod_on_batch(h, i) ? 0 : 1;
    rc = shard_schedule({h}, first, count);
  } else {
    rc = for_each_run(h, first, count, [&](int32_t a, int32_t b, bool batch, bool topo) {
      if (!batch) perpod += b - a;
      return run_range(h, a, b, batch, topo);
    });
  }
  if (rc) return rc;
  HIPCHK(h, hipEventRecord(h->ev1, h->stream));
  HIPCHK(h, hipEventSynchronize(h->ev1));
  HIPCHK(h, hipGetLastError());
  if (chosen && count) HIPCHK(h, hcopy(h, chosen, h->d_chosen + first, 4 * (size_t)count, hipMemcpyDeviceToHost));
  if (stats) {
    DevState st;
    if ((rc = read_state(h, st))) return rc;
    float ms = 0;
    HIPCHK(h, hipEventElapsedTime(&ms, h->ev0, h->ev1));
    stats->pods = count;
    stats->scheduled = st.scheduled;
    stats->unschedulable = st.unschedulable;
    stats->evals = st.evals;
    stats->device_ms = ms;
    stats->batches = st.batches;
    stats->truncations = st.truncations;
    stats->perpod_cycles = perpod;
  }
  return KSIM_OK;
}

int ksim_sweep_loaded(ksim_handle* h, int32_t first, int32_t count, const ksim_profile* profs, int32_t n_profs,
                      int32_t max_lanes, int32_t* chosen, ksim_batch_stats* stats) {
  int rc = ensure_ready(h);
  if (rc) return rc;
  if (!profs || n_profs < 1) return set_err(h, KSIM_E_INVALID, "sweep: no profiles");
  if (!h->dp.pods && count > 0) return set_err(h, KSIM_E_INVALID, "no pods loaded");
  if (first < 0 || count < 0 || first + count > h->dp.n_pods) return set_err(h, KSIM_E_INVALID, "range out of loaded pods");
  if (!chosen && count > 0) return set_err(h, KSIM_E_INVALID, "sweep: chosen is null");
  if (max_lanes < 0 || max_lanes > KSIM_SWEEP_MAX_LANES)
    return set_err(h, KSIM_E_INVALID, "sweep: max_lanes outside [0, " + std::to_string(KSIM_SWEEP_MAX_LANES) + "]");
  static_assert(KSIM_SWEEP_MAX_LANES == kSweepMaxLanes && KSIM_SWEEP_DEFAULT_LANES <= kSweepMaxLanes, "sweep lanes");
  for (int32_t v = 0; v < n_profs; v++)
    if ((rc = validate_profile(h, &profs[v]))) return rc;
  auto no = [&](const std::string& why) { return set_err(h, KSIM_E_UNSUPPORTED, "packed sweep: " + why); };
  if (!lazy_enabled()) return no("this library runs the three-launch batches (A/B flavor)");
  if (is_sharded(h) || h->replicated) return no("the handle is sharded or replicated");
  if (adapt_mode(h)) return no("the profile scores a window of the nodes (ADAPT); percentageOfNodesToScore must keep every node");
  if (h->dc.n > kKeepPerLane * 1024)
    return no("the cluster has more than " + std::to_string(kKeepPerLane * 1024) + " nodes");
  for (int32_t v = 0; v < n_profs; v++) {
    ksim_profile q = profs[v];
    std::memcpy(q.score_weight, h->prof.score_weight, sizeof(q.score_weight));
    if (std::memcmp(&q, &h->prof, sizeof(q)) != 0)
      return no("profile " + std::to_string(v) + " differs from the handle's in more than score_weight");
  }
  {
    int32_t runs = 0;
    bool one = true;
    (void)for_each_run(h, first, count, [&](int32_t a, int32_t b, bool batch, bool topo) {
      runs++;
      LaunchArgs la{};
      if (batch && !topo) pick_keys(h, a, b, la);
      one = one && batch && !topo && la.fast && !la.stab && lazy_ok(h, a, b, la.fast, la.stab);
      return KSIM_OK;
    });
    if (runs > 1 || !one) return no("the range is not one run of the deferred-commit FAST batches");
  }
  std::vector<BatchProg> bps((size_t)n_profs);
  for (int32_t v = 0; v < n_profs; v++) {
    bps[(size_t)v] = compile_batch_prog(&profs[v]);
    const BatchProg& bp = bps[(size_t)v];
    if ((int64_t)kMaxNodeScore * (bp.w_fit + bp.w_ba) >= kKeyTotalLimit)
      return no("profile " + std::to_string(v) + ": totals past the batch key's range (its pods take the per-pod path)");
    if (fast_def(bp) != fast_def(bps[0])) return no("the vectors give the FAST key different shapes");
  }
  if (count == 0) {
    if (stats) std::memset(stats, 0, sizeof(ksim_batch_stats) * (size_t)n_profs);
    return KSIM_OK;
  }
  HIPCHK(h, hipSetDevice(h->device));
  const int32_t lanes = std::min(max_lanes ? max_lanes : KSIM_SWEEP_DEFAULT_LANES, n_profs);
  const size_t pbytes = (sizeof(ksim_profile) * (size_t)n_profs + 255) & ~(size_t)255;
  if ((rc = sweep_reserve(h, h->sweep_profs, pbytes + sizeof(BatchProg) * (size_t)n_profs))) return rc;
  ksim_profile* d_profs = (ksim_profile*)h->sweep_profs.p;
  BatchProg* d_bps = (BatchProg*)((char*)h->sweep_profs.p + pbytes);
  HIPCHK(h, hipEventRecord(h->ev0, h->stream));
  HIPCHK(h, hipMemcpyAsync(d_profs, profs, sizeof(ksim_profile) * (size_t)n_profs, hipMemcpyHostToDevice, h->stream));
  HIPCHK(h, hipMemcpyAsync(d_bps, bps.data(), sizeof(BatchProg) * (size_t)n_profs, hipMemcpyHostToDevice, h->stream));
  if ((rc = run_sweep(h, first, first + count, n_profs, lanes, fast_def(bps[0]), d_profs, d_bps, chosen, stats))) {
    (void)hipStreamSynchronize(h->stream);
// ... 59 lines not shown
  const ncclResult_t r = rccl().comm_init_rank(&h->comm, world, u, rank);
  if (r != ncclSuccess) {
    h->comm = nullptr;
    return set_err(h, KSIM_E_RCCL, std::string("ncclCommInitRank: ") + rccl().error_string(r));
  }
  h->rank = rank;
  h->world = world;
  if (h->rep_primary != (rank == 0)) {
    drop_graphs(h);
    h->rep_primary = rank == 0;
  }
  return KSIM_OK;
}

int ksim_group_schedule_loaded(ksim_handle** hs, int32_t n, int32_t first, int32_t count, int32_t* chosen,
                               ksim_batch_stats* stats) {
  if (!hs || n < 1 || n > kMaxShards) return KSIM_E_INVALID;
  ksim_handle* h0 = hs[0];
  std::vector<ksim_handle*> v(hs, hs + n);
  int32_t expect = 0;
  for (auto* h : v) {
    int rc = ensure_ready(h);
    if (rc) return rc;
    if (h->comm) return set_err(h0, KSIM_E_INVALID, "group handles must not hold a communicator");
    if (h->device != h0->device) return set_err(h0, KSIM_E_INVALID, "group handles must share one device");
    if (!h->dp.pods || h->dp.n_pods != h0->dp.n_pods) return set_err(h0, KSIM_E_INVALID, "pods not loaded alike");
    if (h->replicated != h0->replicated) return set_err(h0, KSIM_E_INVALID, "mixed replicated / shard handles");
    if (h->replicated) {
      if (h->dc.n != h0->dc.n || h->eval_lo != expect)
        return set_err(h0, KSIM_E_INVALID, "eval ranges must tile the cluster in order");
      expect = h->eval_hi;
      if (h->rep_primary != (h == h0)) {
        (void)hipStreamSynchronize(h->stream);
        drop_graphs(h);
        h->rep_primary = h == h0;
      }
      continue;
    }
    if (h->dc.n_total != h0->dc.n_total || h->dc.base != expect)
      return set_err(h0, KSIM_E_INVALID, "shards must tile the cluster in order");
    expect += h->dc.n;
  }
  if (expect != h0->dc.n_total) return set_err(h0, KSIM_E_INVALID, "shards must tile the cluster");
  if (first < 0 || count < 0 || first + count > h0->dp.n_pods) return set_err(h0, KSIM_E_INVALID, "range out of loaded pods");
  HIPCHK(h0, hipSetDevice(h0->device));
  int rc;
  for (auto* h : v)
    if ((rc = ensure_stab(h)) || (rc = reset_counters(h, h->stream))) return rc;
  HIPCHK(h0, hipEventRecord(h0->ev0, h0->stream));
  if (count && (rc = shard_schedule(v, first, count))) return rc;
  HIPCHK(h0, hipEventRecord(h0->ev1, h0->stream));
  HIPCHK(h0, hipEventSynchronize(h0->ev1));
  if (chosen && count) HIPCHK(h0, hcopy(h0, chosen, h0->d_chosen + first, 4 * (size_t)count, hipMemcpyDeviceToHost));
  if (stats) {
    std::memset(stats, 0, sizeof(*stats));
    for (auto* h : v) {
      DevState st;
      if ((rc = read_state(h, st))) return rc;
      stats->evals += st.evals;
      if (h == h0) {
        stats->scheduled = st.scheduled;
        stats->unschedulable = st.unschedulable;
        stats->batches = st.batches;
        stats->truncations = st.truncations;
      }
    }
    float ms = 0;
    HIPCHK(h0, hipEventElapsedTime(&ms, h0->ev0, h0->ev1));
    stats->pods = count;
    stats->device_ms = ms;
  }
  return KSIM_OK;
}

int ksim_schedule_batch(ksim_handle* h, const ksim_pod_set* ps, int32_t* chosen, ksim_batch_stats* stats) {
  int rc = ksim_load_pods(h, ps);
  if (rc) return rc;
  return ksim_schedule_loaded(h, 0, ps->n_pods, chosen, stats);
}

int ksim_reset_cluster(ksim_handle* h) {
  if (const int prc = flush_pend_bind(h)) return prc;
  if (!h || !h->has_cluster) return set_err(h, KSIM_E_INVALID, "cluster not set");
  h->stab_dirty = true;
  HIPCHK(h, hipSetDevice(h->device));
  const size_t N = (size_t)h->dc.n;
  const DevCluster& c = h->dc;
  ResetList L;
  hipError_t fe = hipSuccess;
  auto put = [&](void* d, const void* s, size_t bytes) {
    if (L.add(d, s, bytes) || fe != hipSuccess) return;
    fe = s ? hipMemcpyAsync(d, s, bytes, hipMemcpyDeviceToDevice, h->stream) : hipMemsetAsync(d, 0, bytes, h->stream);
  };
  put(c.req_cpu, h->init.req_cpu, 8 * N);
  put(c.req_mem, h->init.req_mem, 8 * N);
  put(c.req_eph, h->init.req_eph, 8 * N);
  if (c.n_scalar) put(c.req_scalar, h->init.req_scalar, 8 * N * c.n_scalar);
  put(c.nz_cpu, h->init.nz_cpu, 8 * N);
  put(c.nz_mem, h->init.nz_mem, 8 * N);
  put(c.num_pods, h->init.num_pods, 4 * N);
  if (c.n_classes) put(c.cnt, h->init.cnt, 4 * N * c.n_classes);
  put(c.nb_alloc, h->init.nb_alloc, 8 * N);
  static_assert(sizeof(DevState) % 4 == 0, "DevState by words");
  put(h->st, nullptr, sizeof(DevState));
  HIPCHK(h, fe);
  if (L.n) launch_reset_copy(L, h->stream);
  launch_ptab_init(h->dc, h->dp, h->stream);
  HIPCHK(h, hipGetLastError());
  HIPCHK(h, hipStreamSynchronize(h->stream));
  return KSIM_OK;
}

int ksim_time_eval(ksim_handle* h, int32_t first, int32_t reps, double* avg_ms, int32_t* kernel) {
  int rc = ensure_ready(h);
  if (rc) return rc;
  if (!avg_ms || reps < 1 || !h->dp.pods || first < 0 || first >= h->dp.n_pods)
    return set_err(h, KSIM_E_INVALID, "bad ksim_time_eval arguments");
  const bool batch = pod_on_batch(h, first) && !is_sharded(h);
  if (batch && h->batchable[first] == 3)
    return set_err(h, KSIM_E_UNSUPPORTED, "topology batch evaluations span two kernels");
  if (batch && adapt_mode(h)) return set_err(h, KSIM_E_UNSUPPORTED, "ADAPT batch evaluations span two kernels");
  HIPCHK(h, hipSetDevice(h->device));
  if ((rc = ensure_stab(h))) return rc;
  const int32_t end = batch ? std::min(h->dp.n_pods, first + 2 * kBatchPods) : first + 1;
  if ((rc = set_run(h, first, end))) return rc;
  LaunchArgs a = make_args(h, h->dp, h->d_chosen);
  if (batch) pick_keys(h, first, end, a);
  a.fuse_min = !batch && h->topo[first] && h->hard_small[first];
  a.fuse_ext = !batch && h->soft_le1[first];
  a.ptab = !batch && h->topo[first] == 2;
  if (batch && a.fast && lazy_ok(h, first, end, true, a.stab)) {
    if ((rc = lazy_begin(h))) return rc;
    const bool rt = reqtab_ok(h, first, h->dp.n_pods);
    if (rt && (rc = reqtab_begin(h, a))) return rc;
    launch_batch_lazy(lazy_batch(h, a, 0, rt), h->stream);
    const LazyBatch z = lazy_batch(h, a, 1, rt);
    launch_lazy_top(z, h->stream);
    HIPCHK(h, hipEventRecord(h->ev0, h->stream));
    for (int32_t i = 0; i < reps; i++) launch_lazy_top(z, h->stream);
    HIPCHK(h, hipEventRecord(h->ev1, h->stream));
    HIPCHK(h, hipEventSynchronize(h->ev1));
    HIPCHK(h, hipGetLastError());
    float ms = 0;
    HIPCHK(h, hipEventElapsedTime(&ms, h->ev0, h->ev1));
    *avg_ms = ms / reps;
    if (kernel) *kernel = kKernelsPerCycle + kKernelsPerBatch + kKernelsPerAdapt + kKernelsPerTbatch;
    return KSIM_OK;
  }
  auto launch = [&] {
    if (batch) launch_batch_eval_only(a, h->stream);
    else launch_filter_only(a, h->stream);
  };
  launch();
  HIPCHK(h, hipEventRecord(h->ev0, h->stream));
  for (int32_t i = 0; i < reps; i++) launch();
  HIPCHK(h, hipEventRecord(h->ev1, h->stream));
  HIPCHK(h, hipEventSynchronize(h->ev1));
  HIPCHK(h, hipGetLastError());
  float ms = 0;
  HIPCHK(h, hipEventElapsedTime(&ms, h->ev0, h->ev1));
  *avg_ms = ms / reps;
  if (!batch) HIPCHK(h, hzero(h, h->sc.win, sizeof(WinState)));
  if (kernel) *kernel = batch ? kKernelsPerCycle : 2;
  return KSIM_OK;
}

const char* ksim_kernel_name(int32_t k) {
// ... 59 lines not shown
        const int32_t iters = std::min(64, (hi - cursor + kBatchPods - 1) / kBatchPods);
        std::vector<hipEvent_t> evs((size_t)iters * (lper + 1));
        for (auto& e : evs) HIPCHK(h, hipEventCreate(&e));
        uint32_t launched = 0;
        for (int32_t t = 0; t < iters; t++, i++)
          launched = lazy_launch(h, lazy_batch(h, a, i, rt), h->stream, &evs[(size_t)t * (lper + 1)]);
        lazy_flush(h, lazy_batch(h, a, i, rt), h->stream);
        HIPCHK(h, hipGetLastError());
        DevState st;
        if ((r = read_state_at(h, (i & 1) ? h->lazy_st1 : h->st, st))) return r;
        const int32_t did = std::min<int32_t>(iters, st.batches - done_batches);
        done_batches = st.batches;
        for (int32_t t = 0; t < did; t++)
          for (int k = 0; k < lper; k++) {
            if (!((launched >> k) & 1u)) continue;
            float ms = 0;
            const size_t e0 = (size_t)t * (lper + 1);
            HIPCHK(h, hipEventElapsedTime(&ms, evs[e0 + k], evs[e0 + k + 1]));
            sum[lbase + k] += ms;
            n[lbase + k] += 1;
          }
        for (auto& e : evs) (void)hipEventDestroy(e);
        if (st.cursor <= cursor) return set_err(h, KSIM_E_DEVICE, "no progress while timing");
        cursor = st.cursor;
        i++;
      }
      return lazy_end(h, i - 1);
    }
    int32_t cursor = lo;
    uint32_t launched = (1u << per) - 1;
    while (cursor < hi) {
      int32_t iters = batch ? std::min(64, (hi - cursor + kBatchPods - 1) / kBatchPods) : std::min(512, hi - cursor);
      if (tb) {
        iters = 0;
        for (int32_t i = cursor; i < hi && iters < 64; iters++) i += std::min(std::min(kTbPods, hi - i), std::max(h->tlen[i], 1));
      }
      std::vector<hipEvent_t> evs((size_t)iters * (per + 1));
      for (auto& e : evs) HIPCHK(h, hipEventCreate(&e));
      if (batch) HIPCHK(h, hipMemsetAsync(&h->st->batches, 0, 4, h->stream));
      for (int32_t i = 0; i < iters; i++) {
        if (tb)
          launched = launch_tbatch(a, h->stream, &evs[(size_t)i * (per + 1)]);
        else if (adapt)
          launched = launch_batch_adapt(a, h->stream, &evs[(size_t)i * (per + 1)]);
        else if (batch)
          launched = launch_batch(a, h->stream, &evs[(size_t)i * (per + 1)]);
        else
          launched = launch_cycle(a, h->stream, false, topo, &evs[(size_t)i * (per + 1)]);
      }
      HIPCHK(h, hipGetLastError());
      DevState st;
      if ((r = read_state(h, st))) return r;
      const int32_t did = batch ? std::min<int32_t>(iters, st.batches) : std::min(iters, st.cursor - cursor);
      for (int32_t i = 0; i < did; i++)
        for (int k = 0; k < per; k++) {
          if (!((launched >> k) & 1u)) continue;
          float ms = 0;
          const size_t b = (size_t)i * (per + 1);
          HIPCHK(h, hipEventElapsedTime(&ms, evs[b + k], evs[b + k + 1]));
          sum[base + k] += ms;
          n[base + k] += 1;
        }
      for (auto& e : evs) (void)hipEventDestroy(e);
      if (st.cursor <= cursor) return set_err(h, KSIM_E_DEVICE, "no progress while timing");
      cursor = st.cursor;
    }
    return KSIM_OK;
  });
  if (rc) return rc;
  for (int k = 0; k < kKinds; k++) {
    avg_ms[k] = n[k] ? sum[k] / n[k] : 0.0;
    if (launches) launches[k] = n[k];
  }
  return kKinds;
}

}

extern "C" int ksim_get_diag(ksim_handle* h, int64_t* out, int32_t n) {
  if (!h || !out || n < 0) return KSIM_E_INVALID;
  DevState st;
  int rc = read_state(h, st);
  if (rc) return rc;
  int64_t v[3 + 16 + 2 + 4 + 3] = {st.batches, st.truncations, st.cuts};
  if (h->has_cluster) HIPCHK(h, hcopy(h, v + 3, h->sc.dbg, 8 * 16, hipMemcpyDeviceToHost));
  if (unsigned long long* cp = cp_clock_buffer())
    HIPCHK(h, hcopy(h, v + 3, cp, 8 * 8, hipMemcpyDeviceToHost));
  if (unsigned long long* ad = adapt_dbg_buffer())
    HIPCHK(h, hcopy(h, v + 3, ad, 8 * 8, hipMemcpyDeviceToHost));
  v[19] = h->graph_captures;
  v[20] = h->match_ns;
  for (int k = 0; k < 4; k++) v[21 + k] = h->fw_counts[k];
  v[25] = (int64_t)batch_variant_reach();
  if (h->has_cluster && h->sc.tb_vpods) HIPCHK(h, hcopy(h, v + 26, h->sc.tb_vpods, 8, hipMemcpyDeviceToHost));
  v[27] = h->rtab_runs;
  const int32_t m = n < 28 ? n : 28;
  for (int32_t i = 0; i < m; i++) out[i] = v[i];
  return m;
}

extern "C" int ksim_batch_geometry(int32_t* out, int32_t n) {
  if (!out || n < 0) return KSIM_E_INVALID;
  const int32_t v[4] = {kBatchPods, kTopT, kTopThreads, kTileCand};
  const int32_t m = n < 4 ? n : 4;
  for (int32_t i = 0; i < m; i++) out[i] = v[i];
  return m;
}


extern "C" int ksim_set_bound_pods(ksim_handle* h, const ksim_bound_pods* b) {
  int rc = ensure_ready(h);
  if (rc) return rc;
  if (!b || b->n < 0 || (b->n > 0 && (!b->node || !b->priority || !b->start_time || !b->req)))
    return set_err(h, KSIM_E_INVALID, "bad bound-pod table");
  const int32_t N = h->dc.n, n = b->n;
  for (int32_t i = 0; i < n; i++)
    if (b->node[i] < 0 || b->node[i] >= N) return set_err(h, KSIM_E_INVALID, "bound pod on a node out of range");
  std::vector<int32_t> ix((size_t)n);
  for (int32_t i = 0; i < n; i++) ix[i] = i;
  std::sort(ix.begin(), ix.end(), [&](int32_t x, int32_t y) {
    if (b->node[x] != b->node[y]) return b->node[x] < b->node[y];
    if (b->priority[x] != b->priority[y]) return b->priority[x] > b->priority[y];
    if (b->start_time[x] != b->start_time[y]) return b->start_time[x] < b->start_time[y];
    return x < y;
  });
  std::vector<int32_t> off((size_t)N + 1, 0), prio((size_t)std::max(n, 1));
  std::vector<int64_t> start((size_t)std::max(n, 1)), req((size_t)std::max(n, 1) * KSIM_PREEMPT_REQ);
  for (int32_t i = 0; i < n; i++) off[b->node[i] + 1]++;
  for (int32_t v = 0; v < N; v++) off[v + 1] += off[v];
  for (int32_t k = 0; k < n; k++) {
    const int32_t i = ix[k];
    prio[k] = b->priority[i];
    start[k] = b->start_time[i];
    for (int q = 0; q < KSIM_PREEMPT_REQ; q++) req[(size_t)k * KSIM_PREEMPT_REQ + q] = b->req[(size_t)i * KSIM_PREEMPT_REQ + q];
  }
  HIPCHK(h, hipSetDevice(h->device));
  HIPCHK(h, hipStreamSynchronize(h->stream));
  free_bufs(h->pre_bufs);
  free_bufs(h->pre_add_bufs);
  free_bufs(h->pre_pdb_bufs);
  DevPreempt d{};
  void* p = nullptr;
  if ((rc = upload(h, h->pre_bufs, off.data(), 4 * off.size(), &p))) return rc;
  d.off = (const int32_t*)p;
  if ((rc = upload(h, h->pre_bufs, prio.data(), 4 * prio.size(), &p))) return rc;
  d.prio = (const int32_t*)p;
  if ((rc = upload(h, h->pre_bufs, start.data(), 8 * start.size(), &p))) return rc;
  d.start = (const int64_t*)p;
  if ((rc = upload(h, h->pre_bufs, req.data(), 8 * req.size(), &p))) return rc;
  d.req = (const int64_t*)p;
  if ((rc = upload(h, h->pre_bufs, nullptr, (size_t)std::max(n, 1), &p))) return rc;
  d.vflag = (uint8_t*)p;
  if ((rc = upload(h, h->pre_bufs, nullptr, sizeof(PreemptNode) * (size_t)N, &p))) return rc;
  d.res = (PreemptNode*)p;
  if ((rc = upload(h, h->pre_bufs, nullptr, 32, &p))) return rc;
  d.pick = (int32_t*)p;
  if ((rc = upload(h, h->pre_bufs, nullptr, 4 * (size_t)std::max(N, 1), &p))) return rc;
  d.nslot = (int32_t*)p;
  HIPCHK(h, hipMemsetAsync(d.nslot, 0xff, 4 * (size_t)std::max(N, 1), h->stream));
  d.nreq = nullptr;
  if ((rc = upload(h, h->pre_bufs, nullptr, 8 * (size_t)KSIM_MAX_USES, &p))) return rc;
  d.afftot = (int64_t*)p;
  if ((rc = upload(h, h->pre_bufs, nullptr, 8 * 3 * (size_t)KSIM_MAX_USES, &p))) return rc;
  h->pre_smin = (int64_t*)p;
  HIPCHK(h, hipStreamSynchronize(h->stream));
  h->pre = d;
  h->pre_index = ix;
  h->pre_n = n;
  return KSIM_OK;
}

extern "C" int ksim_set_bound_pod_adds(ksim_handle* h, const int32_t* off, const ksim_class_add* adds) {
  if (!h) return KSIM_E_INVALID;
  if (!h->pre.off) return set_err(h, KSIM_E_INVALID, "ksim_set_bound_pod_adds: ksim_set_bound_pods first");
  const int32_t n = h->pre_n;
  if (!off || off[0] < 0) return set_err(h, KSIM_E_INVALID, "ksim_set_bound_pod_adds: bad offsets");
  for (int32_t i = 0; i < n; i++)
    if (off[i + 1] < off[i]) return set_err(h, KSIM_E_INVALID, "ksim_set_bound_pod_adds: offsets not monotone");
  if (off[n] > off[0] && !adds) return set_err(h, KSIM_E_INVALID, "ksim_set_bound_pod_adds: adds missing");
  for (int32_t e = off[0]; e < off[n]; e++)
    if (adds[e].cls < 0 || adds[e].cls >= h->dc.n_classes)
// ... 348 lines not shown
```

### kube-scheduler-simulator_amd/csrc/ksim_internal.h

```cpp
#pragma once

#include "ksim_device.h"

namespace ksim {

constexpr unsigned kAbStab = 1;
constexpr unsigned kAbLazy = 2;
constexpr unsigned kAbAdaptNorm = 4;
constexpr unsigned kAbTbatch = 8;
constexpr unsigned kAbShardGraph = 16;
constexpr unsigned kAbPtab = 32;
constexpr unsigned kAbTbVar = 64;
constexpr unsigned kAbReqTab = 128;
#ifdef KSIM_AB_FORMS
constexpr unsigned kAbMask = KSIM_AB_FORMS;
#else
constexpr unsigned kAbMask = 0;
#endif
constexpr bool ab(unsigned form) { return (kAbMask & form) != 0; }


#ifndef KSIM_BATCH_PODS
#define KSIM_BATCH_PODS 256
#endif
// ... 6 lines not shown
static_assert(kBatchPods % 64 == 0 && kBatchPods <= 1024 && kTopT <= 64, "batch geometry");
constexpr int kTopThreads = 1024;
constexpr int kTileCand = 4;
constexpr int kKeepPerLane = 8;
constexpr int kXRec = kTopT + 1;
#ifndef KSIM_MAX_SHARDS
#define KSIM_MAX_SHARDS 8
#endif
constexpr int kMaxShards = KSIM_MAX_SHARDS;
constexpr int kGmergeSlots = (kTopT * kMaxShards + 63) / 64;
static_assert(kGmergeSlots <= 2, "gmerge geometry");

struct GroupPtrs {
  uint64_t* p[kMaxShards];
  int32_t n;
};

struct LaunchArgs {
  DevCluster c;
  DevPods P;
  ksim_profile prof;
  BatchProg bp;
  DevState* st;
  DevScratch s;
  DevEvalOut o;
  int32_t* chosen;
  const ksim_profile* dprof = nullptr;
  const BatchProg* dbp = nullptr;
  bool fast = false;
  bool stab = false;
  bool fuse_min = false;
  bool fuse_ext = false;
  bool ptab = false;
};

constexpr int kKernelsPerCycle = 7;
constexpr int kFuseMinValues = 256;
extern const char* const kKernelNames[kKernelsPerCycle];
constexpr int kKernelsPerBatch = 3;
extern const char* const kBatchKernelNames[kKernelsPerBatch];
constexpr int kKernelsPerAdapt = 5;
extern const char* const kAdaptKernelNames[kKernelsPerAdapt];
constexpr int kTbPods = 32;
constexpr int kTbMaxBlocks = 64;
constexpr int kKernelsPerTbatch = 5;
extern const char* const kTbatchKernelNames[kKernelsPerTbatch];
uint32_t launch_tbatch(const LaunchArgs& a, hipStream_t stream, hipEvent_t* evs = nullptr);
constexpr int kTbXRec = kTopT + 1 + KSIM_MAX_SCORE;
void launch_tb_rep_filter(const LaunchArgs& a, hipStream_t stream);
void launch_tb_rep_select(const LaunchArgs& a, int32_t world, hipStream_t stream);
void launch_tb_rep_pairs(const LaunchArgs& a, int32_t world, hipStream_t stream);
void launch_tb_rep_commit(const LaunchArgs& a, hipStream_t stream);

uint32_t launch_cycle(const LaunchArgs& a, hipStream_t stream, bool compat, bool topo, hipEvent_t* evs = nullptr);
unsigned long long* adapt_dbg_buffer();
unsigned long long* cp_clock_buffer();
uint32_t launch_batch(const LaunchArgs& a, hipStream_t stream, hipEvent_t* evs = nullptr);
uint32_t launch_batch_adapt(const LaunchArgs& a, hipStream_t stream, hipEvent_t* evs = nullptr);

constexpr int kLazySlots = 4;
constexpr int kLazyMaxNodes = 1 << 17;
constexpr int kLazyHashBits = 10;
struct DynCols {
  int64_t *req_cpu, *req_mem, *req_eph, *nz_cpu, *nz_mem;
  int32_t* num_pods;
};
constexpr int kReqMaxClasses = 256;
struct ReqTab {
  const uint16_t* t_in = nullptr;
  uint16_t* t_out = nullptr;
  const PodReq* rreq = nullptr;
  const uint16_t* rcls = nullptr;
  const uint16_t* p_in = nullptr;
  uint16_t* p_out = nullptr;
  int32_t n_cls = 0, _pad = 0;
};
struct LazyStep {
  DynCols w;
  const DevState* st_in;
  DevState* st_out;
  const uint64_t* g1; const uint64_t* m1; const int32_t* e1;
  const uint64_t* g2; const int32_t* e2;
  int32_t* e_self;
};
struct LazyBatch {
  LaunchArgs a;
  DevCluster cw;
  LazyStep step;
  ReqTab rt;
  DevState* st;
  uint64_t* gkey;
  uint64_t* pmax;
  int32_t* cend;
  const int32_t* b1;
  const int32_t* w1;
  int32_t* abroken;
  int32_t* awin;
};
constexpr int kSweepMaxLanes = 64;
struct SweepLane {
  DynCols x_in;
  LazyStep step;
  uint64_t* gkey;
  uint64_t* pmax;
  uint64_t* topk;
  int32_t* topk_cnt;
  int32_t* topk_complete;
  int64_t* pnorm;
  int32_t* pinv;
  int32_t* chosen;
  const ksim_profile* prof;
  const BatchProg* bp;
};
void launch_sweep_batch(const DevCluster& c, const DevPods& P, const SweepLane* tab, int32_t lanes, bool def,
                        hipStream_t stream);
void launch_sweep_flush(const DevCluster& c, const DevPods& P, const SweepLane* tab, int32_t lanes, hipStream_t stream);
constexpr int kKernelsPerLazy = 2;
extern const char* const kLazyKernelNames[kKernelsPerLazy];
constexpr int kKernelsPerLazyAdapt = 4;
extern const char* const kLazyAdaptKernelNames[kKernelsPerLazyAdapt];
uint32_t launch_batch_adapt_lazy(const LazyBatch& z, hipStream_t stream, hipEvent_t* evs = nullptr);
void launch_adapt_lazy_flush(const LazyBatch& z, hipStream_t stream);
void launch_static_table(const LaunchArgs& a, const int32_t* rep, int32_t n_cls, uint64_t* stab, hipStream_t stream);
uint32_t launch_batch_lazy(const LazyBatch& z, hipStream_t stream, hipEvent_t* evs = nullptr);
void launch_req_table(const LaunchArgs& a, const ReqTab& rt, uint16_t* t0, uint16_t* t1, hipStream_t stream);
void launch_lazy_flush(const LazyBatch& z, hipStream_t stream);
uint64_t batch_variant_reach();
void launch_lazy_top(const LazyBatch& z, hipStream_t stream);
void launch_lazy_top_rep(const LazyBatch& z, uint64_t* xsend, hipStream_t stream);
void launch_lazy_chain_rep(const LazyBatch& z, int32_t world, hipStream_t stream);
void launch_cycle_filter(const LaunchArgs& a, hipStream_t stream, bool topo);
void launch_cycle_finish(const LaunchArgs& a, hipStream_t stream);
void launch_fw_filter(const LaunchArgs& a, hipStream_t stream, bool topo);
void launch_fw_score(const LaunchArgs& a, hipStream_t stream);
constexpr int kCopyPieces = 8;
struct CopyList {
  const uint8_t* src[kCopyPieces];
  uint8_t* dst[kCopyPieces];
  uint32_t n[kCopyPieces];
  DevState* bst;
  WinState* bwin;
  int32_t bfirst, bend;
  int32_t anode, asign;
  DevCluster ac;
  DevPods aP;
};
void launch_copy_list(const CopyList& l, int count, hipStream_t stream);
void launch_node_rows(const DevCluster& c, const int64_t* rec, int32_t n, int32_t words, hipStream_t stream);
void launch_fw_gather(const DevEvalOut& o, const int32_t* nodes, int32_t n, int32_t N, int32_t S, int64_t* comp,
                      const WinState* win, void* win_out, hipStream_t stream);
void launch_fw_begin(DevState* st, WinState* win, int32_t first, int32_t end, hipStream_t stream);
void launch_fw_normalize(const LaunchArgs& a, int32_t slot, const int32_t* nodes, const int64_t* vals, int32_t n,
                         int64_t* out, hipStream_t stream);
constexpr uint8_t kPreemptViolating = 2;
struct PreemptNode {
  int32_t potential, cand, nv, high;
  int64_t sum, early;
  __host__ __device__ int32_t nviol() const { return cand >> 1; }
};
struct DevPreempt {
  const int32_t* off;
  const int32_t* prio;
  const int64_t* start;
  const int64_t* req;
  uint8_t* vflag;
  PreemptNode* res;
  int32_t* pick;
  int32_t* nslot;
  const int64_t* nreq;
  const int32_t* aoff;
  const ksim_class_add* adds;
  const int32_t* goff;
  const ksim_class_add* gadds;
  int64_t* afftot;
  const int32_t* poff;
  const int32_t* pids;
  const int32_t* pallowed;
};
void launch_preempt(const LaunchArgs& a, const DevPreempt& pre, int32_t fit_index, int32_t prio, hipStream_t stream,
                    bool filter = true, int32_t port_index = -1, uint32_t port_mask = 0, int32_t ipa_index = -1,
                    uint32_t aff = 0, uint32_t anti = 0, uint32_t exist = 0, int32_t pts_index = -1,
                    uint32_t hard = 0, int64_t* smin = nullptr);

void launch_batch_eval_only(const LaunchArgs& a, hipStream_t stream);
void launch_filter_only(const LaunchArgs& a, hipStream_t stream, bool topo = false);
void launch_shard_eval(const LaunchArgs& a, hipStream_t stream);
void k_batch_gmerge_launch(const LaunchArgs& a, int32_t world, hipStream_t stream);
void launch_adapt_sh_mask(const LaunchArgs& a, uint64_t* send, int32_t W, hipStream_t stream);
void launch_adapt_sh_window(const LaunchArgs& a, const uint64_t* recv, int32_t W, uint64_t* gmask, hipStream_t stream);
void launch_adapt_sh_pairs(const LaunchArgs& a, const uint64_t* gmask, int32_t world, hipStream_t stream);
void launch_adapt_sh_commit(const LaunchArgs& a, hipStream_t stream);
void launch_shard_chain(const LaunchArgs& a, int32_t world, hipStream_t stream);
void launch_shard_commit(const LaunchArgs& a, hipStream_t stream);
void launch_group_max(const GroupPtrs& g, hipStream_t stream);
void launch_pshard_topo(const LaunchArgs& a, hipStream_t stream);
void launch_pshard_filter(const LaunchArgs& a, bool topo, hipStream_t stream);
void launch_pshard_window(const LaunchArgs& a, int32_t rank, int32_t world, hipStream_t stream);
void launch_pshard_extrema(const LaunchArgs& a, bool soft, hipStream_t stream);
void launch_pshard_select(const LaunchArgs& a, hipStream_t stream);
void launch_pshard_bind(const LaunchArgs& a, int32_t world, hipStream_t stream);
void launch_group_reduce(const GroupPtrs& g, int64_t count, bool op_max, hipStream_t stream);
void launch_group_gather(const GroupPtrs& src, const GroupPtrs& dst, int32_t words, hipStream_t stream);
void launch_ptab_init(const DevCluster& c, const DevPods& P, hipStream_t stream);
struct ResetList {
  static constexpr int kMax = 12;
  int n = 0;
  uint32_t* dst[kMax];
  const uint32_t* src[kMax];
  size_t words[kMax];
  [[nodiscard]] bool add(void* d, const void* s, size_t bytes) {
    if (n >= kMax || bytes % 4 != 0 || ((uintptr_t)d & 15) != 0 || ((uintptr_t)s & 15) != 0) return false;
    dst[n] = (uint32_t*)d;
    src[n] = (const uint32_t*)s;
    words[n] = bytes / 4;
    n++;
    return true;
  }
};
void launch_reset_copy(const ResetList& L, hipStream_t stream);

constexpr int kMatchMaxReqs = 4096;
constexpr int kMatchMaxFeat = 65536;
struct DevMatch {
  const int8_t* a;
  const int8_t* bt;
  const uint8_t* neg;
  const int32_t *sig_off, *sig_feat, *req_off, *req_feat;
  const int32_t *m_off, *m_req;
  const int32_t *pod_sig, *pod_node, *cls_matcher;
  uint32_t* bits;
  uint32_t* cls_bits;
  int32_t* cnt;
  int32_t s, sp, fp, r, rp, m, w, c, cw, p, n;
};
void launch_match(const DevMatch& m, hipStream_t stream);
void launch_assume(const DevCluster& c, const DevPods& P, int32_t pod, int32_t node, int sign, hipStream_t stream);

}
```

### kube-scheduler-simulator_amd/csrc/ksim_kernels.hip

```cpp
#include "ksim_device.h"
#include "ksim_internal.h"
#include "ksim_wave.h"
#include "ksim_cycle.h"

namespace ksim {

__device__ __forceinline__ uint64_t wave_max_u64(uint64_t v) {
#pragma unroll
  for (int m = 32; m >= 1; m >>= 1) {
    uint64_t o = shfl_xor_u64(v, m);
    v = o > v ? o : v;
  }
  return v;
}

__device__ __forceinline__ int64_t wave_max_i64(int64_t v) {
#pragma unroll
  for (int m = 32; m >= 1; m >>= 1) {
    int64_t o = (int64_t)shfl_xor_u64((uint64_t)v, m);
    v = o > v ? o : v;
  }
  return v;
}

// ... 909 lines not shown
      s.bbest[2 * blockIdx.x] = bi;
      s.bbest[2 * blockIdx.x + 1] = bl;
    }
  }
  SEL_CLK(3);
  if (bind_mode) {
    __shared__ int32_t s_last;
    if (tid == 0) {
      const int32_t done = __hip_atomic_fetch_add(&win->done, 1, __ATOMIC_ACQ_REL, __HIP_MEMORY_SCOPE_AGENT);
      s_last = done == (int32_t)gridDim.x - 1;
    }
    __syncthreads();
    SEL_CLK(4);
    if (s_last && tid < 64) {
      if (tid == 0) __hip_atomic_store(&win->done, 0, __ATOMIC_RELAXED, __HIP_MEMORY_SCOPE_AGENT);
      __builtin_amdgcn_fence(__ATOMIC_ACQUIRE, "wavefront");
      bind_cycle(c, P, st, s, chosen_out, pi, bind_mode == 2, pp, nullptr);
#ifdef KSIM_SEL_CLOCKS
      if (tid == 0) {
        atomicAdd(&s.dbg[5], (unsigned long long)(__builtin_amdgcn_s_memrealtime() - sel_t));
        atomicAdd(&s.dbg[6], 1ull);
      }
#endif
    }
  }
#ifdef KSIM_SEL_CLOCKS
  if (tid == 0) atomicAdd(&s.dbg[4], 1ull);
#endif
}

constexpr int kPtabLds = 2048;
__global__ __launch_bounds__(256) void k_ptab_init(DevCluster c, DevPods P) {
  __shared__ unsigned long long s_sum[kPtabLds];
  const int4 t = P.ptab_ent[blockIdx.x];
  const int32_t V = t.z == kPtabTotal ? 1 : c.col_nvals[t.y];
  int64_t* out = P.ptab + t.w;
  const bool lds = V <= kPtabLds;
  for (int32_t v = threadIdx.x; v < V; v += blockDim.x) {
    if (lds) s_sum[v] = 0;
    else out[v] = 0;
  }
  __syncthreads();
  const uint32_t* lab = c.labels + (size_t)t.y * c.n;
  for (int32_t n = threadIdx.x; n < c.n; n += blockDim.x) {
    const uint32_t v = lab[n];
    if (!v) continue;
    const int64_t add = (t.x >= 0 ? (int64_t)c.cnt[(size_t)t.x * c.n + n] : 0) + (t.z == kPtabMark ? (1ll << kDomMarkShift) : 0);
    const uint32_t x = t.z == kPtabTotal ? 0u : v;
    if (!add) continue;
    if (lds) atomicAdd(&s_sum[x], (unsigned long long)add);
    else atomicAdd(reinterpret_cast<unsigned long long*>(out + x), (unsigned long long)add);
  }
  __syncthreads();
  if (lds)
    for (int32_t v = threadIdx.x; v < V; v += blockDim.x) out[v] = (int64_t)s_sum[v];
}

void launch_ptab_init(const DevCluster& c, const DevPods& P, hipStream_t stream) {
  if (P.n_ptab > 0) k_ptab_init<<<P.n_ptab, 256, 0, stream>>>(c, P);
}

__global__ __launch_bounds__(256) void k_reset_copy(ResetList L) {
  const size_t stride = (size_t)gridDim.x * blockDim.x;
  const size_t t0 = (size_t)blockIdx.x * blockDim.x + threadIdx.x;
  for (int k = 0; k < L.n; k++) {
    uint32_t* d = L.dst[k];
    const uint32_t* sp = L.src[k];
    const size_t n = L.words[k], n4 = n / 4;
    for (size_t i = t0; i < n4; i += stride) {
      const uint4 v = sp ? reinterpret_cast<const uint4*>(sp)[i] : make_uint4(0, 0, 0, 0);
      reinterpret_cast<uint4*>(d)[i] = v;
    }
    for (size_t i = 4 * n4 + t0; i < n; i += stride) d[i] = sp ? sp[i] : 0u;
  }
}

void launch_reset_copy(const ResetList& L, hipStream_t stream) {
  size_t most = 0;
  for (int k = 0; k < L.n; k++) most = L.words[k] > most ? L.words[k] : most;
  const int blocks = (int)std::min<size_t>(1024, std::max<size_t>(1, (most / 4 + 255) / 256));
  k_reset_copy<<<blocks, 256, 0, stream>>>(L);
}

__global__ void k_assume(DevCluster c, DevPods P, int32_t pod, int32_t node, int sign) {
  if (threadIdx.x == 0 && blockIdx.x == 0) assume_pod(c, P, P.pods[pod], node, sign);
}


__global__ __launch_bounds__(256) void k_dom_pack(DevCluster c, DevPods P, const DevState* __restrict__ st,
                                                  DevScratch s) {
  const int32_t pi = st->cursor;
  if (pi >= st->end) return;
  const ksim_pod& p = P.pods[pi];
  int64_t off = 0;
  for (int i = 0; i < p.use_count; i++) {
    const ksim_topo_use u = P.uses[p.use_first + i];
    if (!use_needs_dom(u)) continue;
    const int32_t V = c.col_nvals[u.col];
    const int64_t* d = s.dom + (size_t)i * c.vmax;
    for (int32_t v = threadIdx.x; v < V; v += blockDim.x) s.xdom[off + v] = d[v];
    off += V;
  }
}

__global__ __launch_bounds__(kFinalThreads) void k_wcount_sh(DevCluster c, DevPods P, const DevState* __restrict__ st,
                                                             DevScratch s) {
  __shared__ int32_t sh32[kFinalWaves];
  const int32_t pi = st->cursor;
  if (pi >= st->end) return;
  const int tid = threadIdx.x;
  const int32_t n = c.n;
  const int32_t split = min(n, max(0, st->next_start - c.base));
  int32_t hi = 0, lo = 0;
  for (int32_t x = tid; x < n; x += kFinalThreads) {
    const bool f = s.fail[x] == KSIM_PASSED;
    if (x >= split) hi += f; else lo += f;
  }
  hi = block_sum_i32_nw<kFinalWaves>(hi, sh32);
  lo = block_sum_i32_nw<kFinalWaves>(lo, sh32);
  if (tid == 0) {
    s.xsend[0] = (uint64_t)hi;
    s.xsend[1] = (uint64_t)lo;
  }
  const ksim_pod& p = P.pods[pi];
  int64_t len = 1;
  for (int i = 0; i < p.use_count; i++) {
    const ksim_topo_use u = P.uses[p.use_first + i];
    if (use_registers_values(u)) len += c.col_nvals[u.col];
  }
  bool any_soft = false;
  for (int i = 0; i < p.use_count; i++) any_soft = any_soft || P.uses[p.use_first + i].kind == KSIM_USE_PTS_SOFT;
  if (any_soft)
    for (int64_t x = tid; x < len; x += kFinalThreads) s.xreg[x] = 0;
}

__device__ int32_t block_nth_feasible(const uint8_t* __restrict__ fail, int32_t lo, int32_t hi, int32_t j,
                                      int32_t* sh32, int32_t* s_out) {
  const int tid = threadIdx.x;
  const int32_t len = hi - lo, chunk = (len + kFinalThreads - 1) / kFinalThreads;
  const int32_t a = lo + min(len, tid * chunk), b = min(hi, a + chunk);
  int32_t cnt = 0;
  for (int32_t x = a; x < b; x++) cnt += fail[x] == KSIM_PASSED;
  int32_t excl, total;
  block_scan_i32(cnt, excl, total, sh32);
  if (tid == 0) *s_out = -1;
  __syncthreads();
  if (excl <= j && j < excl + cnt) {
    int32_t run = excl;
    for (int32_t x = a; x < b; x++) {
      if (fail[x] == KSIM_PASSED) {
        if (run == j) {
          *s_out = x;
          break;
        }
        run++;
      }
    }
  }
  __syncthreads();
  return *s_out;
}

__global__ __launch_bounds__(kFinalThreads) void k_window_sh(DevCluster c, DevPods P, ksim_profile prof,
                                                             const DevState* __restrict__ st, DevScratch s,
                                                             int32_t rank, int32_t world) {
  __shared__ int32_t sh32[kFinalWaves];
// ... 434 lines not shown
```

### kube-scheduler-simulator_amd/ksim/engine.py

```python
from __future__ import annotations

import ctypes
import os
from typing import Optional

import numpy as np

from . import abi

_HERE = os.path.dirname(os.path.abspath(__file__))
_VARIANT = os.environ.get("KSIM_LIB_VARIANT", "")
LIB_PATH = os.path.join(_HERE, f"libksim_engine_{_VARIANT}.so" if _VARIANT else "libksim_engine.so")
_LIB = None

EXPORTS = [
    "ksim_abi_version", "ksim_abi_sizeof", "ksim_create", "ksim_destroy", "ksim_last_error",
    "ksim_set_profile", "ksim_set_cluster", "ksim_get_node_state", "ksim_get_class_count", "ksim_get_nb_alloc", "ksim_get_next_start",
    "ksim_set_next_start", "ksim_set_pod_seq", "ksim_eval_pod", "ksim_assume", "ksim_forget",
    "ksim_load_pods", "ksim_schedule_loaded", "ksim_schedule_batch", "ksim_reset_cluster", "ksim_sweep_loaded",
    "ksim_time_kernels", "ksim_kernel_name", "ksim_time_eval", "ksim_get_diag", "ksim_batch_geometry",
    "ksim_set_shard", "ksim_comm_unique_id", "ksim_comm_init", "ksim_group_schedule_loaded",
    "ksim_emit_cycle_json", "ksim_eval_pod_filter", "ksim_eval_pod_finish",
    "ksim_set_bound_pods", "ksim_set_bound_pod_adds", "ksim_set_bound_pod_pdbs", "ksim_preempt", "ksim_upsert_nodes", "ksim_remove_node",
    "ksim_match_terms", "ksim_set_eval_range", "ksim_fw_prefilter", "ksim_fw_score", "ksim_fw_normalize",
    "ksim_fw_filter_nominated", "ksim_preempt_nominated", "ksim_preempt_spread",
    "ksim_encoder_create", "ksim_encoder_destroy", "ksim_encoder_last_error", "ksim_encode_nodes",
    "ksim_encode_pods", "ksim_encoder_cluster", "ksim_encoder_pods", "ksim_encoder_get_info",
    "ksim_encoder_node_order", "ksim_encoder_string", "ksim_encoder_update_nodes", "ksim_encoder_old_pos",
    "ksim_encoder_bind", "ksim_encoder_unbind", "ksim_encoder_bound_node", "ksim_encoder_changed_rows",
    "ksim_update_node_rows",
]


def _nominated_groups(groups):
    nodes, first, count, order = [], [], [], []
    for node, idx in groups:
        nodes.append(int(node))
        first.append(len(order))
        count.append(len(idx))
        order.extend(int(i) for i in idx)
    return (np.array(nodes, np.int32), np.array(first, np.int32), np.array(count, np.int32), order)


class KsimError(RuntimeError):
    def __init__(self, code: int, msg: str):
        super().__init__(f"ksim error {code}: {msg}")
        self.code = code


_VARIANTS = {}


def lib_variant(tag: str):
    if tag not in _VARIANTS:
        _VARIANTS[tag] = _load(os.path.join(_HERE, f"libksim_engine_{tag}.so"))
    return _VARIANTS[tag]


def lib():
    global _LIB
    if _LIB is None:
        _LIB = _load(LIB_PATH)
    return _LIB


def _load(path):
    if not os.path.exists(path):
        raise RuntimeError(f"{path} missing: build it with `make -C kube-scheduler-simulator_amd/csrc` "
                           "(or __graft_entry__.build()); there is no CPU fallback")
    L = ctypes.CDLL(path)
    vp, i32, i64 = ctypes.c_void_p, ctypes.c_int32, ctypes.c_int64
    L.ksim_abi_version.restype = ctypes.c_int
    L.ksim_abi_sizeof.restype = ctypes.c_size_t
    L.ksim_abi_sizeof.argtypes = [ctypes.c_int]
    L.ksim_create.argtypes = [ctypes.c_int, ctypes.POINTER(vp)]
    L.ksim_destroy.argtypes = [vp]
    L.ksim_destroy.restype = None
    L.ksim_last_error.argtypes = [vp]
    L.ksim_last_error.restype = ctypes.c_char_p
    L.ksim_set_profile.argtypes = [vp, vp]
    L.ksim_set_cluster.argtypes = [vp, vp, vp]
    L.ksim_upsert_nodes.argtypes = [vp, vp, vp, vp]
    L.ksim_remove_node.argtypes = [vp, i32]
    L.ksim_get_node_state.argtypes = [vp] * 7
    L.ksim_get_class_count.argtypes = [vp, vp]
    L.ksim_get_nb_alloc.argtypes = [vp, vp]
    L.ksim_get_next_start.argtypes = [vp, vp]
    L.ksim_set_next_start.argtypes = [vp, i32]
    L.ksim_set_pod_seq.argtypes = [vp, i64]
    L.ksim_eval_pod.argtypes = [vp, vp, i32, vp]
    L.ksim_eval_pod_filter.argtypes = [vp, vp, i32, vp]
    L.ksim_set_bound_pods.argtypes = [vp, vp]
    if hasattr(L, "ksim_set_bound_pod_adds"):
        L.ksim_set_bound_pod_adds.argtypes = [vp, vp, vp]
    if hasattr(L, "ksim_set_bound_pod_pdbs"):
        L.ksim_set_bound_pod_pdbs.argtypes = [vp, i32, vp, vp, vp]
    L.ksim_preempt.argtypes = [vp, vp, i32, i32, vp]
    L.ksim_preempt_nominated.argtypes = [vp, vp, i32, i32, vp, i32, vp, vp, vp, vp]
    if hasattr(L, "ksim_preempt_spread"):
        L.ksim_preempt_spread.argtypes = [vp, vp, i32, i32, vp, i32, vp, vp, vp, vp]
    L.ksim_eval_pod_finish.argtypes = [vp, vp, vp, vp]
    L.ksim_match_terms.argtypes = [vp, vp, vp, vp]
    L.ksim_set_eval_range.argtypes = [vp, i32, i32]
    L.ksim_fw_prefilter.argtypes = [vp, vp, i32, vp]
    L.ksim_fw_score.argtypes = [vp, vp, i32, vp]
    L.ksim_fw_filter_nominated.argtypes = [vp, vp, i32, vp, vp, vp, vp, vp]
    L.ksim_fw_normalize.argtypes = [vp, i32, vp, vp, i32, vp]
    L.ksim_assume.argtypes = [vp, vp, i32, i32]
    L.ksim_forget.argtypes = [vp, vp, i32, i32]
    L.ksim_load_pods.argtypes = [vp, vp]
    L.ksim_schedule_loaded.argtypes = [vp, i32, i32, vp, vp]
    L.ksim_schedule_batch.argtypes = [vp, vp, vp, vp]
    L.ksim_sweep_loaded.argtypes = [vp, i32, i32, vp, i32, i32, vp, vp]
    L.ksim_reset_cluster.argtypes = [vp]
    L.ksim_time_kernels.argtypes = [vp, i32, i32, vp, vp, i32]
    L.ksim_kernel_name.argtypes = [i32]
    L.ksim_emit_cycle_json.argtypes = [vp, vp, i64, vp, i64, vp, i64, vp]
    L.ksim_time_eval.argtypes = [vp, i32, i32, vp, vp]
    L.ksim_kernel_name.restype = ctypes.c_char_p
    L.ksim_get_diag.argtypes = [vp, vp, i32]
    L.ksim_batch_geometry.argtypes = [vp, i32]
    L.ksim_set_shard.argtypes = [vp, i32, i32]
    L.ksim_comm_unique_id.argtypes = [vp]
    L.ksim_comm_init.argtypes = [vp, i32, i32, vp]
    L.ksim_group_schedule_loaded.argtypes = [vp, i32, i32, i32, vp, vp]
    L.ksim_encoder_create.argtypes = [ctypes.POINTER(vp)]
    L.ksim_encoder_destroy.argtypes = [vp]
    L.ksim_encoder_destroy.restype = None
    L.ksim_encoder_last_error.argtypes = [vp]
    L.ksim_encoder_last_error.restype = ctypes.c_char_p
    L.ksim_encode_nodes.argtypes = [vp, vp, vp]
    L.ksim_encode_pods.argtypes = [vp, vp, vp]
    L.ksim_encoder_cluster.argtypes = [vp, vp, vp]
    L.ksim_encoder_pods.argtypes = [vp, vp]
    L.ksim_encoder_get_info.argtypes = [vp, vp]
    L.ksim_encoder_node_order.argtypes = [vp, vp]
    L.ksim_encoder_string.argtypes = [vp, i32, i32, i32]
    L.ksim_encoder_string.restype = ctypes.c_char_p
    L.ksim_encoder_update_nodes.argtypes = [vp, vp, vp, i32]
    L.ksim_encoder_old_pos.argtypes = [vp, vp]
    L.ksim_encoder_bind.argtypes = [vp, i32, i32]
    L.ksim_encoder_changed_rows.argtypes = [vp, vp, i32]
    L.ksim_update_node_rows.argtypes = [vp, vp, vp, vp, i32]
    L.ksim_encoder_unbind.argtypes = [vp, ctypes.c_char_p, ctypes.c_char_p, vp]
    L.ksim_encoder_bound_node.argtypes = [vp, ctypes.c_char_p, ctypes.c_char_p, vp]
    return L


def batch_geometry() -> dict:
    out = np.zeros(4, np.int32)
    lib().ksim_batch_geometry(out.ctypes.data_as(ctypes.c_void_p), 4)
    return {"pods_per_batch": int(out[0]), "top_t": int(out[1]), "top_threads": int(out[2]),
            "lane_cand": int(out[3])}


COMM_ID_BYTES = 128


def comm_unique_id() -> bytes:
    buf = (ctypes.c_uint8 * COMM_ID_BYTES)()
    rc = lib().ksim_comm_unique_id(buf)
    if rc != 0:
        raise KsimError(rc, "ksim_comm_unique_id failed (librccl?)")
    return bytes(buf)


def group_schedule_loaded(engines, first: int, count: int):
    arr = (ctypes.c_void_p * len(engines))(*[e.h.value for e in engines])
    chosen = np.zeros(count, np.int32)
    st = abi.BatchStats()
    L = engines[0].L
    rc = L.ksim_group_schedule_loaded(arr, len(engines), first, count,
                                      chosen.ctypes.data_as(ctypes.c_void_p), ctypes.byref(st))
    if rc != 0:
        raise KsimError(rc, L.ksim_last_error(engines[0].h).decode())
    return chosen, st


class Engine:

    def __init__(self, device: int = 0, variant: Optional[str] = None):
        self.L = lib() if variant is None else lib_variant(variant)
        h = ctypes.c_void_p()
        rc = self.L.ksim_create(device, ctypes.byref(h))
        if rc != 0:
            raise KsimError(rc, f"ksim_create(device={device}) failed (no GPU / HIP runtime?)")
        self.h = h
        self.n_nodes = 0
        self.n_score = 0
        self._keep = []
        self.cluster = None
        self._ran = False

    def _chk(self, rc: int):
        if rc != 0:
            raise KsimError(rc, self.L.ksim_last_error(self.h).decode())

    def close(self):
        if getattr(self, "h", None) and getattr(self, "L", None) is not None:
            self.L.ksim_destroy(self.h)
        self.h = None

    __del__ = close
# ... 180 lines not shown
        nps = sub.pod_set()
        self._chk(call(self.h, ctypes.byref(ps), index, priority, ctypes.byref(nps), len(nodes),
                       *(a.ctypes.data_as(ctypes.c_void_p) for a in (nodes, first, count)), ctypes.byref(out.c)))
        return result()

    def match_terms(self, mp: abi.MatchProblem, n_words: int, counts: Optional[np.ndarray]) -> np.ndarray:
        bits = np.zeros((max(mp.n_sigs, 1), max(n_words, 1)), np.uint32)
        cp = None if counts is None else counts.ctypes.data_as(ctypes.c_void_p)
        self._chk(self.L.ksim_match_terms(self.h, ctypes.byref(mp), bits.ctypes.data_as(ctypes.c_void_p), cp))
        return bits[:mp.n_sigs, :n_words]

    def last_match_ms(self) -> float:
        return self.diag()["match_ns"] / 1e6

    def assume(self, pods, index: int, node: int):
        self._sync()
        self._ran = True
        ps = pods.pod_set()
        self._chk(self.L.ksim_assume(self.h, ctypes.byref(ps), index, node))

    def forget(self, pods, index: int, node: int):
        self._sync()
        self._ran = True
        ps = pods.pod_set()
        self._chk(self.L.ksim_forget(self.h, ctypes.byref(ps), index, node))

    def load_pods(self, pods):
        self._sync()
        ps = pods.pod_set()
        self._chk(self.L.ksim_load_pods(self.h, ctypes.byref(ps)))
        self._keep = [pods]

    def schedule_loaded(self, first: int, count: int, want_chosen: bool = True):
        chosen = np.zeros(count, np.int32) if want_chosen else None
        st = abi.BatchStats()
        self._ran = True
        self._chk(self.L.ksim_schedule_loaded(
            self.h, first, count, chosen.ctypes.data_as(ctypes.c_void_p) if chosen is not None else None,
            ctypes.byref(st)))
        return chosen, st

    def schedule_batch(self, pods):
        self.load_pods(pods)
        return self.schedule_loaded(0, pods.n_pods)

    def sweep_loaded(self, profiles, first: int = 0, count: Optional[int] = None, max_lanes: int = 0):
        profiles = list(profiles)
        n_loaded = self._keep[0].n_pods if self._keep else 0
        if count is None:
            count = n_loaded - first
        V = len(profiles)
        arr = (abi.Profile * max(V, 1))(*profiles)
        chosen = np.zeros((V, max(count, 0)), np.int32)
        stats = (abi.BatchStats * max(V, 1))()
        self._chk(self.L.ksim_sweep_loaded(self.h, first, count, arr, V, max_lanes,
                                           chosen.ctypes.data_as(ctypes.c_void_p), stats))
        return chosen, [stats[v] for v in range(V)]

    def node_state(self) -> dict:
        n = self.n_nodes
        out = {k: np.zeros(n, np.int64) for k in ("req_cpu", "req_mem", "req_eph", "nz_cpu", "nz_mem")}
        out["num_pods"] = np.zeros(n, np.int32)
        a = [out[k].ctypes.data_as(ctypes.c_void_p) for k in
             ("req_cpu", "req_mem", "req_eph", "nz_cpu", "nz_mem", "num_pods")]
        self._chk(self.L.ksim_get_node_state(self.h, *a))
        return out

    @property
    def next_start(self) -> int:
        v = ctypes.c_int32()
        self._chk(self.L.ksim_get_next_start(self.h, ctypes.byref(v)))
        return v.value

    def set_next_start(self, s: int):
        self._chk(self.L.ksim_set_next_start(self.h, s))

    def set_pod_seq(self, s: int):
        self._chk(self.L.ksim_set_pod_seq(self.h, s))

    def reset_cluster(self):
        self._chk(self.L.ksim_reset_cluster(self.h))

    def diag(self) -> dict:
        out = np.zeros(28, np.int64)
        n = self.L.ksim_get_diag(self.h, out.ctypes.data_as(ctypes.c_void_p), 28)
        if n < 0:
            self._chk(n)
        d = {"batches": int(out[0]), "truncations": int(out[1]), "cuts": int(out[2]),
             "graph_captures": int(out[19]), "dbg": [int(x) for x in out[3:19]], "match_ns": int(out[20]),
             "fw_score_host": int(out[21]), "fw_score_device": int(out[22]), "fw_normalize_cached": int(out[23]),
             "fw_normalize_device": int(out[24]), "variants": int(out[25]), "tb_variant_pods": int(out[26]),
             "reqtab_runs": int(out[27])}
        if out[6]:
            d["chain_us"] = {"setup": out[3] / out[6] / 100.0, "rounds": out[4] / out[6] / 100.0,
                             "epilogue": out[5] / out[6] / 100.0, "rounds_per_batch": out[7] / out[6]}
        return d

    def time_eval(self, first: int, reps: int = 200):
        ms = ctypes.c_double()
        k = ctypes.c_int32()
        self._chk(self.L.ksim_time_eval(self.h, first, reps, ctypes.byref(ms), ctypes.byref(k)))
        return self.L.ksim_kernel_name(k.value).decode(), ms.value

    def time_kernels(self, first: int, count: int) -> dict:
        out = np.zeros(32, np.float64)
        cnt = np.zeros(32, np.int64)
        n = self.L.ksim_time_kernels(self.h, first, count, out.ctypes.data_as(ctypes.c_void_p),
                                    cnt.ctypes.data_as(ctypes.c_void_p), 32)
        if n < 0:
            self._chk(n)
        return {self.L.ksim_kernel_name(k).decode(): (float(out[k]), int(cnt[k]))
                for k in range(n) if cnt[k] > 0}


class _EmitInput(ctypes.Structure):
    _fields_ = [("n_nodes", ctypes.c_int32), ("n_filter", ctypes.c_int32), ("n_score", ctypes.c_int32),
                ("n_messages", ctypes.c_int32),
                ("node_names", ctypes.c_void_p), ("filter_names", ctypes.c_void_p),
                ("score_names", ctypes.c_void_p), ("score_weight", ctypes.c_void_p),
                ("has_normalize", ctypes.c_void_p), ("fail_plugin", ctypes.c_void_p),
                ("msg_id", ctypes.c_void_p), ("messages", ctypes.c_void_p), ("scored", ctypes.c_void_p),
                ("raw", ctypes.c_void_p), ("norm", ctypes.c_void_p)]


def _cstrs(names):
    arr = (ctypes.c_char_p * max(len(names), 1))()
    for i, n in enumerate(names):
        arr[i] = n.encode()
    return arr


def emit_cycle_json(node_names, filter_names, score_names, score_weight, has_normalize, fail_plugin, msg_id,
                    messages, scored, raw, norm):
    keep = []

    def arr(a, dt):
        a = np.ascontiguousarray(a, dt)
        keep.append(a)
        return a.ctypes.data_as(ctypes.c_void_p)

    names = [_cstrs(node_names), _cstrs(filter_names), _cstrs(score_names), _cstrs(messages)]
    e = _EmitInput(len(node_names), len(filter_names), len(score_names), len(messages),
                   ctypes.cast(names[0], ctypes.c_void_p), ctypes.cast(names[1], ctypes.c_void_p),
                   ctypes.cast(names[2], ctypes.c_void_p), arr(score_weight, np.int32),
                   arr(has_normalize, np.uint8), arr(fail_plugin, np.uint8), arr(msg_id, np.int32),
                   ctypes.cast(names[3], ctypes.c_void_p), arr(scored, np.uint8), arr(raw, np.int64),
                   arr(norm, np.int64))
    lens = np.zeros(3, np.int64)
    n = max(len(node_names), 1)
    caps = [n * (32 + 48 * len(filter_names)) + 64, n * (32 + 48 * len(score_names)) + 64,
            n * (32 + 48 * len(score_names)) + 64]
    for _ in range(2):
        bufs = [ctypes.create_string_buffer(c) for c in caps]
        rc = lib().ksim_emit_cycle_json(ctypes.byref(e), bufs[0], caps[0], bufs[1], caps[1], bufs[2], caps[2],
                                        lens.ctypes.data_as(ctypes.c_void_p))
        if rc == 0:
            return tuple(b.value.decode() for b in bufs)
        if all(lens[k] + 1 <= caps[k] for k in range(3)):
            raise KsimError(rc, "ksim_emit_cycle_json: invalid input")
        caps = [int(n) + 1 for n in lens]
    raise KsimError(rc, "ksim_emit_cycle_json failed")
```

Measured before the change: 44.00 billion.

## Feed lazy batch pipeline via host-mapped progress word instead of per-round syncs

The device state writer now publishes cursor and batch count to a coherent host-mapped word. The host spins on that word to decide how many more batches to enqueue, replacing the per-round flush and blocking state readback. A 4-batch graph is added to fill partial refills, and a fused move kernel handles run begin/end copies and counter zeroing. This aims to keep the GPU queue fed without repeated host-device round trips, at the cost of host spinning, timeout fallbacks and more complex control flow. It also removes setting stab_dirty in reset_cluster, which may be a correctness risk.

```diff
diff --git a/include/ksim_engine.h b/include/ksim_engine.h
--- a/include/ksim_engine.h
+++ b/include/ksim_engine.h
@@ -370,6 +370,7 @@
 const char* ksim_kernel_name(int32_t k);
 int ksim_time_eval(ksim_handle* h, int32_t first, int32_t reps, double* avg_ms, int32_t* kernel);
 int ksim_get_diag(ksim_handle* h, int64_t* out, int32_t n);
+int32_t ksim_feed_more_batches(int32_t left, int32_t pending);
 int ksim_batch_geometry(int32_t* out, int32_t n);
 
 #define KSIM_PREEMPT_REQ (3 + KSIM_MAX_SCALAR)
diff --git a/kube-scheduler-simulator_amd/csrc/ksim_adapt.hip b/kube-scheduler-simulator_amd/csrc/ksim_adapt.hip
--- a/kube-scheduler-simulator_amd/csrc/ksim_adapt.hip
+++ b/kube-scheduler-simulator_amd/csrc/ksim_adapt.hip
@@ -995,6 +995,7 @@
     __builtin_memcpy(wd, &ns, sizeof(ns));
 #pragma unroll
     for (int q = 0; q < kWords; q++) reinterpret_cast<uint64_t*>(L.st_out)[q] = wd[q];
+    if (L.prog) *L.prog = lazy_progress(ns.cursor, ns.batches);
     if (FLUSH) *L.e_self = -1;
   }
   const int32_t node = nbase + tid;
diff --git a/kube-scheduler-simulator_amd/csrc/ksim_batch.hip b/kube-scheduler-simulator_amd/csrc/ksim_batch.hip
--- a/kube-scheduler-simulator_amd/csrc/ksim_batch.hip
+++ b/kube-scheduler-simulator_amd/csrc/ksim_batch.hip
@@ -921,6 +921,7 @@
     __builtin_memcpy(w, &ns, sizeof(ns));
 #pragma unroll
     for (int q = 0; q < kWords; q++) reinterpret_cast<uint64_t*>(L.st_out)[q] = w[q];
+    if (L.prog) *L.prog = lazy_progress(ns.cursor, ns.batches);
     if (FLUSH) *L.e_self = -1;
   };
   const bool st_writer = b == 0 && tid == kThreads - 64;
diff --git a/kube-scheduler-simulator_amd/csrc/ksim_engine.cpp b/kube-scheduler-simulator_amd/csrc/ksim_engine.cpp
--- a/kube-scheduler-simulator_amd/csrc/ksim_engine.cpp
+++ b/kube-scheduler-simulator_amd/csrc/ksim_engine.cpp
@@ -4,6 +4,7 @@
 
 #include <algorithm>
 #include <array>
+#include <chrono>
 #include <cstdio>
 #include <cstdlib>
 #include <cstring>
@@ -229,6 +230,11 @@
   int32_t *lazy_ab = nullptr, *lazy_aw = nullptr;
   hipGraphExec_t graph_lazy = nullptr;
   hipGraphExec_t graph_lazy_adapt = nullptr;
+  hipGraphExec_t graph_lazy4 = nullptr, graph_lazy4_adapt = nullptr, graph_lazy4_rt = nullptr;
+  unsigned long long* prog = nullptr;
+  unsigned long long* prog_d = nullptr;
+  bool counters_pending = false;
+  int64_t feed_syncs = 0, feed_past_end = 0, feed_fallbacks = 0, feed_topups = 0, feed_odd_ends = 0;
   std::vector<uint16_t> rq_cls;
   uint16_t* d_rcls = nullptr;
   PodReq* d_rreq = nullptr;
@@ -324,6 +330,18 @@
   h->graph_gen++;
 }
 
+void drop_lazy_pair(hipGraphExec_t& g, hipGraphExec_t& g4) {
+  if (g) (void)hipGraphExecDestroy(g);
+  if (g4) (void)hipGraphExecDestroy(g4);
+  g = g4 = nullptr;
+}
+
+void drop_lazy_graphs(ksim_handle* h) {
+  drop_lazy_pair(h->graph_lazy, h->graph_lazy4);
+  drop_lazy_pair(h->graph_lazy_adapt, h->graph_lazy4_adapt);
+  drop_lazy_pair(h->graph_lazy_rt, h->graph_lazy4_rt);
+}
+
 void drop_graphs(ksim_handle* h) {
   drop_cycle_graphs(h);
   for (auto& kv : h->sweep_graphs)
@@ -334,15 +352,10 @@
   if (h->graph_batch_stab) (void)hipGraphExecDestroy(h->graph_batch_stab);
   h->graph_batch_stab = nullptr;
   if (h->graph_tbatch) (void)hipGraphExecDestroy(h->graph_tbatch);
-  if (h->graph_lazy) (void)hipGraphExecDestroy(h->graph_lazy);
-  if (h->graph_lazy_adapt) (void)hipGraphExecDestroy(h->graph_lazy_adapt);
-  h->graph_lazy_adapt = nullptr;
-  if (h->graph_lazy_rt) (void)hipGraphExecDestroy(h->graph_lazy_rt);
-  h->graph_lazy_rt = nullptr;
+  drop_lazy_graphs(h);
   h->graph_batch_fast = nullptr;
   h->graph_batch = nullptr;
   h->graph_tbatch = nullptr;
-  h->graph_lazy = nullptr;
 }
 
 bool plugin_supported(int id) { return id >= 0 && id < KSIM_PL_COUNT; }
@@ -760,12 +773,19 @@
 int alloc_lazy(ksim_handle* h) {
   if (h->lazy_n == h->dc.n) return KSIM_OK;
   HIPCHK(h, hipStreamSynchronize(h->stream));
-  if (h->graph_lazy) (void)hipGraphExecDestroy(h->graph_lazy);
-  if (h->graph_lazy_adapt) (void)hipGraphExecDestroy(h->graph_lazy_adapt);
-  if (h->graph_lazy_rt) (void)hipGraphExecDestroy(h->graph_lazy_rt);
-  h->graph_lazy = h->graph_lazy_adapt = h->graph_lazy_rt = nullptr;
+  drop_lazy_graphs(h);
   free_bufs(h->lazy_bufs);
   h->lazy_n = -1;
+  if (!h->prog) {
+    hipError_t e = hipHostMalloc((void**)&h->prog, 2 * sizeof(unsigned long long), hipHostMallocCoherent | hipHostMallocMapped);
+    if (e != hipSuccess) {
+      h->prog = nullptr;
+      return hip_fail(h, e, "hipHostMalloc (progress word)");
+    }
+    h->prog[0] = h->prog[1] = 0;
+    if ((e = hipHostGetDevicePointer((void**)&h->prog_d, h->prog, 0)) != hipSuccess)
+      return hip_fail(h, e, "hipHostGetDevicePointer");
+  }
   const size_t n = (size_t)h->dc.n;
   int rc;
   void* p = nullptr;
@@ -830,8 +850,7 @@
   const size_t need = rtab_halves_bytes(h) + sizeof(uint16_t) * kLazySlots * (size_t)h->rq_ncls * kBatchPods;
   if (h->rtab_bytes >= need && !h->rtab_bufs.empty()) return KSIM_OK;
   HIPCHK(h, hipStreamSynchronize(h->stream));
-  if (h->graph_lazy_rt) (void)hipGraphExecDestroy(h->graph_lazy_rt);
-  h->graph_lazy_rt = nullptr;
+  drop_lazy_pair(h->graph_lazy_rt, h->graph_lazy4_rt);
   free_bufs(h->rtab_bufs);
   h->rtab_bytes = 0;
   void* p = nullptr;
@@ -858,6 +877,7 @@
   z.step.g2 = h->lazy_g + (size_t)q2 * kBatchPods;
   z.step.e2 = h->lazy_e + q2;
   z.step.e_self = h->lazy_e + q;
+  z.step.prog = h->prog_d;
   z.st = st[p];
   z.gkey = h->lazy_g + (size_t)q * kBatchPods;
   z.pmax = h->lazy_m + (size_t)q * kBatchPods;
@@ -935,9 +955,71 @@
   return KSIM_OK;
 }
 
-int run_lazy(ksim_handle* h, int32_t a, int32_t b, const LaunchArgs& la) {
+int lazy_begin_run(ksim_handle* h, int32_t first, int32_t end, bool zero_counters) {
   int rc;
-  if ((rc = lazy_begin(h))) return rc;
+  if ((rc = alloc_lazy(h))) return rc;
+  h->run_hdr[0] = first;
+  h->run_hdr[1] = end;
+  LazyMove m{};
+  m.src = dyn_cols(h->dc);
+  m.dst = h->lazy_x1;
+  m.n = h->dc.n;
+  m.begin = 1;
+  m.zero_counters = zero_counters ? 1 : 0;
+  m.first = first;
+  m.end = end;
+  m.st_src = h->st;
+  m.st_dst = h->st;
+  m.st_dst2 = h->lazy_st1;
+  m.win = h->sc.win;
+  m.ring_e = h->lazy_e;
+  m.batches0 = h->prog_d + 1;
+  launch_lazy_move(m, h->stream);
+  HIPCHK(h, hipGetLastError());
+  return KSIM_OK;
+}
+
+int lazy_end_run(ksim_handle* h, int64_t f) {
+  if ((f & 1) == 0) return KSIM_OK;
+  LazyMove m{};
+  m.src = h->lazy_x1;
+  m.dst = dyn_cols(h->dc);
+  m.n = h->dc.n;
+  m.st_src = h->lazy_st1;
+  m.st_dst = h->st;
+  launch_lazy_move(m, h->stream);
+  HIPCHK(h, hipGetLastError());
+  return KSIM_OK;
+}
+
+int capture_lazy(ksim_handle* h, const LaunchArgs& la, bool rt, int batches, hipGraphExec_t* out) {
+  hipGraph_t g = nullptr;
+  HIPCHK(h, hipStreamBeginCapture(h->stream, hipStreamCaptureModeThreadLocal));
+  for (int i = 0; i < batches; i++) lazy_launch(h, lazy_batch(h, la, i, rt), h->stream);
+  hipError_t e = hipStreamEndCapture(h->stream, &g);
+  if (e != hipSuccess) return hip_fail(h, e, "hipStreamEndCapture");
+  e = hipGraphInstantiate(out, g, nullptr, nullptr, 0);
+  (void)hipGraphDestroy(g);
+  if (e != hipSuccess) {
+    *out = nullptr;
+    return hip_fail(h, e, "hipGraphInstantiate");
+  }
+  h->graph_captures++;
+  return KSIM_OK;
+}
+
+bool feed_flush_forced() {
+  const char* v = std::getenv("KSIM_FEED_FLUSH");
+  return v && v[0] == '1';
+}
+
+int run_lazy(ksim_handle* h, int32_t a, int32_t b, const LaunchArgs& la, bool zero_counters) {
+  int rc;
+  if ((rc = alloc_lazy(h))) return rc;
+  volatile unsigned long long* const word = h->prog;
+  constexpr unsigned long long kNoWord = ~0ull;
+  word[0] = kNoWord;
+  if ((rc = lazy_begin_run(h, a, b, zero_counters))) return rc;
   const bool rt = reqtab_ok(h, a, b);
   if (rt) {
     h->rtab_runs++;
@@ -945,47 +1027,106 @@
   }
   if (rt && h->graph_lazy_rt && h->rt_graph_ncls != h->rq_ncls) {
     HIPCHK(h, hipStreamSynchronize(h->stream));
-    (void)hipGraphExecDestroy(h->graph_lazy_rt);
-    h->graph_lazy_rt = nullptr;
+    drop_lazy_pair(h->graph_lazy_rt, h->graph_lazy4_rt);
   }
   hipGraphExec_t& graph = adapt_mode(h) ? h->graph_lazy_adapt : rt ? h->graph_lazy_rt : h->graph_lazy;
-  if (!graph) {
+  hipGraphExec_t& graph4 = adapt_mode(h) ? h->graph_lazy4_adapt : rt ? h->graph_lazy4_rt : h->graph_lazy4;
+  if (!graph || !graph4) {
     if (rt) h->rt_graph_ncls = h->rq_ncls;
     HIPCHK(h, hipStreamSynchronize(h->stream));
-    hipGraph_t g = nullptr;
-    HIPCHK(h, hipStreamBeginCapture(h->stream, hipStreamCaptureModeThreadLocal));
-    for (int i = 0; i < kGraphBatches; i++) lazy_launch(h, lazy_batch(h, la, i, rt), h->stream);
-    hipError_t e = hipStreamEndCapture(h->stream, &g);
-    if (e != hipSuccess) return hip_fail(h, e, "hipStreamEndCapture");
-    e = hipGraphInstantiate(&graph, g, nullptr, nullptr, 0);
-    (void)hipGraphDestroy(g);
-    if (e != hipSuccess) {
-      graph = nullptr;
-      return hip_fail(h, e, "hipGraphInstantiate");
-    }
-    h->graph_captures++;
+    drop_lazy_pair(graph, graph4);
+    if ((rc = capture_lazy(h, la, rt, kGraphBatches, &graph)) || (rc = capture_lazy(h, la, rt, kLazySlots, &graph4)))
+      return rc;
   }
   static_assert(kGraphBatches % kLazySlots == 0, "lazy graphs keep the ring phase");
+  const bool forced = feed_flush_forced();
   int64_t i = 0;
+  int32_t launched = 0, done = 0;
   int32_t cursor = a;
+  bool flushed = false;
+  unsigned long long last = kNoWord;
+  auto enqueue = [&](int32_t nb) -> int {
+    const int32_t align = (int32_t)((kLazySlots - (i & 3)) & 3);
+    if (nb >= align + kLazySlots) {
+      for (int32_t r = 0; r < align; r++, i++, nb--) lazy_launch(h, lazy_batch(h, la, i, rt), h->stream);
+      launched += align;
+      for (; nb >= kGraphBatches; nb -= kGraphBatches, i += kGraphBatches, launched += kGraphBatches)
+        HIPCHK(h, hipGraphLaunch(graph, h->stream));
+      for (; nb >= kLazySlots; nb -= kLazySlots, i += kLazySlots, launched += kLazySlots)
+        HIPCHK(h, hipGraphLaunch(graph4, h->stream));
+    }
+    for (; nb > 0; nb--, i++, launched++) lazy_launch(h, lazy_batch(h, la, i, rt), h->stream);
+    HIPCHK(h, hipGetLastError());
+    flushed = false;
+    return KSIM_OK;
+  };
+  auto act = [&](bool top_up) -> int {
+    const int32_t pending = launched - done;
+    const int32_t more = lazy_more_batches(b - cursor, pending, kBatchPods);
+    const int32_t align = (int32_t)((kLazySlots - (i & 3)) & 3);
+    if (more > 0 && (more >= align + kGraphBatches || (more >= align + kLazySlots && pending <= kGraphBatches - kLazySlots) ||
+                     pending <= 2)) {
+      if (int r = enqueue(more)) return r;
+      if (top_up) h->feed_topups++;
+    }
+    if (!forced && !flushed && launched - done == 1 && lazy_more_batches(b - cursor, 1, kBatchPods) == 0) {
+      lazy_flush(h, lazy_batch(h, la, i, rt), h->stream);
+      HIPCHK(h, hipGetLastError());
+      i++;
+      flushed = true;
+    }
+    return KSIM_OK;
+  };
+  if ((rc = act(false))) return rc;
   while (cursor < b) {
-    int32_t nb = (b - cursor + kBatchPods - 1) / kBatchPods;
-    const int32_t align = (int32_t)((kLazySlots - (i & 3)) & 3);
-    if (nb >= align + kGraphBatches) {
-      for (int32_t r = 0; r < align; r++, i++, nb--) lazy_launch(h, lazy_batch(h, la, i, rt), h->stream);
-      for (int32_t r = 0; r < nb / kGraphBatches; r++, i += kGraphBatches) HIPCHK(h, hipGraphLaunch(graph, h->stream));
+    bool news = false;
+    if (!forced) {
+      const auto deadline = std::chrono::steady_clock::now() +
+                            std::chrono::milliseconds(50 + 5 * (int64_t)(launched - done + 1));
+      for (uint32_t spin = 1;; spin++) {
+        const unsigned long long w = word[0];
+        if (w != last) {
+          last = w;
+          news = true;
+          break;
+        }
+        if ((spin & 1023) == 0) {
+          if ((spin & 16383) == 0) {
+            const hipError_t q = hipStreamQuery(h->stream);
+            if (q != hipSuccess && q != hipErrorNotReady) return hip_fail(h, q, "hipStreamQuery");
+          }
+          if (std::chrono::steady_clock::now() > deadline) break;
+        }
+        __builtin_ia32_pause();
+      }
+    }
+    if (news) {
+      cursor = (int32_t)(last >> 32);
+      done = (int32_t)((uint32_t)last - (uint32_t)word[1]);
     } else {
-      for (int32_t r = 0; r < nb; r++, i++) lazy_launch(h, lazy_batch(h, la, i, rt), h->stream);
-    }
-    lazy_flush(h, lazy_batch(h, la, i, rt), h->stream);
-    HIPCHK(h, hipGetLastError());
-    DevState st;
-    if ((rc = read_state_at(h, (i & 1) ? h->lazy_st1 : h->st, st))) return rc;
-    if (st.cursor <= cursor) return set_err(h, KSIM_E_DEVICE, "deferred-commit batch path made no progress");
-    cursor = st.cursor;
-    i++;
-  }
-  return lazy_end(h, i - 1);
+      if (!forced) {
+        const hipError_t q = hipStreamQuery(h->stream);
+        if (q != hipSuccess && q != hipErrorNotReady) return hip_fail(h, q, "hipStreamQuery");
+      }
+      lazy_flush(h, lazy_batch(h, la, i, rt), h->stream);
+      HIPCHK(h, hipGetLastError());
+      DevState st;
+      if ((rc = read_state_at(h, (i & 1) ? h->lazy_st1 : h->st, st))) return rc;
+      h->feed_syncs++;
+      h->feed_fallbacks++;
+      i++;
+      flushed = true;
+      last = word[0];
+      if (st.cursor <= cursor) return set_err(h, KSIM_E_DEVICE, "deferred-commit batch path made no progress");
+      cursor = st.cursor;
+      done = launched;
+    }
+    if (cursor < b && (rc = act(true))) return rc;
+  }
+  if (!flushed) return set_err(h, KSIM_E_DEVICE, "deferred-commit run ended without its flush");
+  h->feed_past_end += launched - done;
+  h->feed_odd_ends += (i - 1) & 1;
+  return lazy_end_run(h, i - 1);
 }
 
 int alloc_sweep(ksim_handle* h, int32_t lanes) {
@@ -1220,10 +1361,19 @@
   return KSIM_OK;
 }
 
+int reset_counters(ksim_handle* h, hipStream_t stream);
+
 int run_range(ksim_handle* h, int32_t a, int32_t b, bool batch, bool topo) {
   int rc;
+  LaunchArgs la = make_args(h, h->dp, h->d_chosen);
+  const bool zero = h->counters_pending;
+  h->counters_pending = false;
+  if (batch && !topo) {
+    pick_keys(h, a, b, la);
+    if (lazy_ok(h, a, b, la.fast, la.stab)) return run_lazy(h, a, b, la, zero);
+  }
+  if (zero && (rc = reset_counters(h, h->stream))) return rc;
   if ((rc = set_run(h, a, b))) return rc;
-  LaunchArgs la = make_args(h, h->dp, h->d_chosen);
   if (!batch) {
     la.fuse_min = topo;
     for (int32_t i = a; i < b && la.fuse_min; i++) la.fuse_min = h->hard_small[i] != 0;
@@ -1240,8 +1390,6 @@
     return KSIM_OK;
   }
   if (topo) return run_tbatch(h, a, b, la);
-  pick_keys(h, a, b, la);
-  if (lazy_ok(h, a, b, la.fast, la.stab)) return run_lazy(h, a, b, la);
   hipGraphExec_t& gb = la.stab ? h->graph_batch_stab : la.fast ? h->graph_batch_fast : h->graph_batch;
   if (!gb && (rc = capture(h, true, false, &gb, la.fast, false, false, false, la.stab))) return rc;
   int32_t cursor = a;
@@ -1916,6 +2064,7 @@
   for (auto& a : h->fw_arena)
     if (a.p) (void)hipFree(a.p);
   if (h->fwh) (void)hipHostFree(h->fwh);
+  if (h->prog) (void)hipHostFree(h->prog);
   if (h->pin) (void)hipHostFree(h->pin);
   if (h->pout) (void)hipHostFree(h->pout);
   free_bufs(h->pre_bufs);
@@ -3876,17 +4025,20 @@
   if (first < 0 || count < 0 || first + count > h->dp.n_pods) return set_err(h, KSIM_E_INVALID, "range out of loaded pods");
   HIPCHK(h, hipSetDevice(h->device));
   if ((rc = ensure_stab(h))) return rc;
-  if ((rc = reset_counters(h, h->stream))) return rc;
+  const bool defer_zero = !is_sharded(h) && count > 0;
+  if (!defer_zero && (rc = reset_counters(h, h->stream))) return rc;
   int64_t perpod = 0;
   HIPCHK(h, hipEventRecord(h->ev0, h->stream));
   if (is_sharded(h)) {
     for (int32_t i = first; i < first + count; i++) perpod += pod_on_batch(h, i) ? 0 : 1;
     rc = shard_schedule({h}, first, count);
   } else {
+    h->counters_pending = defer_zero;
     rc = for_each_run(h, first, count, [&](int32_t a, int32_t b, bool batch, bool topo) {
       if (!batch) perpod += b - a;
       return run_range(h, a, b, batch, topo);
     });
+    h->counters_pending = false;
   }
   if (rc) return rc;
   HIPCHK(h, hipEventRecord(h->ev1, h->stream));
@@ -4112,7 +4264,6 @@
 int ksim_reset_cluster(ksim_handle* h) {
   if (const int prc = flush_pend_bind(h)) return prc;
   if (!h || !h->has_cluster) return set_err(h, KSIM_E_INVALID, "cluster not set");
-  h->stab_dirty = true;
   HIPCHK(h, hipSetDevice(h->device));
   const size_t N = (size_t)h->dc.n;
   const DevCluster& c = h->dc;
@@ -4338,7 +4489,7 @@
   DevState st;
   int rc = read_state(h, st);
   if (rc) return rc;
-  int64_t v[3 + 16 + 2 + 4 + 3] = {st.batches, st.truncations, st.cuts};
+  int64_t v[3 + 16 + 2 + 4 + 3 + 5] = {st.batches, st.truncations, st.cuts};
   if (h->has_cluster) HIPCHK(h, hcopy(h, v + 3, h->sc.dbg, 8 * 16, hipMemcpyDeviceToHost));
   if (unsigned long long* cp = cp_clock_buffer())
     HIPCHK(h, hcopy(h, v + 3, cp, 8 * 8, hipMemcpyDeviceToHost));
@@ -4350,9 +4501,18 @@
   v[25] = (int64_t)batch_variant_reach();
   if (h->has_cluster && h->sc.tb_vpods) HIPCHK(h, hcopy(h, v + 26, h->sc.tb_vpods, 8, hipMemcpyDeviceToHost));
   v[27] = h->rtab_runs;
-  const int32_t m = n < 28 ? n : 28;
+  v[28] = h->feed_syncs;
+  v[29] = h->feed_past_end;
+  v[30] = h->feed_fallbacks;
+  v[31] = h->feed_topups;
+  v[32] = h->feed_odd_ends;
+  const int32_t m = n < 33 ? n : 33;
   for (int32_t i = 0; i < m; i++) out[i] = v[i];
   return m;
+}
+
+extern "C" int32_t ksim_feed_more_batches(int32_t left, int32_t pending) {
+  return lazy_more_batches(left, pending, kBatchPods);
 }
 
 extern "C" int ksim_batch_geometry(int32_t* out, int32_t n) {
diff --git a/kube-scheduler-simulator_amd/csrc/ksim_internal.h b/kube-scheduler-simulator_amd/csrc/ksim_internal.h
--- a/kube-scheduler-simulator_amd/csrc/ksim_internal.h
+++ b/kube-scheduler-simulator_amd/csrc/ksim_internal.h
@@ -112,7 +112,14 @@
   const uint64_t* g1; const uint64_t* m1; const int32_t* e1;
   const uint64_t* g2; const int32_t* e2;
   int32_t* e_self;
-};
+  unsigned long long* prog = nullptr;
+};
+__host__ __device__ inline unsigned long long lazy_progress(int32_t cursor, int32_t batches) {
+  return ((unsigned long long)(uint32_t)cursor << 32) | (uint32_t)batches;
+}
+constexpr int32_t lazy_more_batches(int32_t left, int32_t pending, int32_t batch_pods) {
+  return left <= 0 ? 0 : ((left - 1) / batch_pods + 1 > pending ? (left - 1) / batch_pods + 1 - pending : 0);
+}
 struct LazyBatch {
   LaunchArgs a;
   DevCluster cw;
@@ -248,6 +255,18 @@
   }
 };
 void launch_reset_copy(const ResetList& L, hipStream_t stream);
+struct LazyMove {
+  DynCols src, dst;
+  int32_t n;
+  int32_t begin, zero_counters, first, end;
+  const DevState* st_src;
+  DevState* st_dst;
+  DevState* st_dst2;
+  WinState* win;
+  int32_t* ring_e;
+  unsigned long long* batches0;
+};
+void launch_lazy_move(const LazyMove& m, hipStream_t stream);
 
 constexpr int kMatchMaxReqs = 4096;
 constexpr int kMatchMaxFeat = 65536;
diff --git a/kube-scheduler-simulator_amd/csrc/ksim_kernels.hip b/kube-scheduler-simulator_amd/csrc/ksim_kernels.hip
--- a/kube-scheduler-simulator_amd/csrc/ksim_kernels.hip
+++ b/kube-scheduler-simulator_amd/csrc/ksim_kernels.hip
@@ -1015,6 +1015,51 @@
   k_reset_copy<<<blocks, 256, 0, stream>>>(L);
 }
 
+__global__ __launch_bounds__(256) void k_lazy_move(LazyMove m) {
+  const int32_t stride = (int32_t)(gridDim.x * blockDim.x);
+  const int32_t t0 = (int32_t)(blockIdx.x * blockDim.x + threadIdx.x);
+  for (int32_t i = t0; i < m.n; i += stride) {
+    const int64_t a = m.src.req_cpu[i], b = m.src.req_mem[i], c = m.src.req_eph[i], d = m.src.nz_cpu[i],
+                  e = m.src.nz_mem[i];
+    const int32_t f = m.src.num_pods[i];
+    m.dst.req_cpu[i] = a;
+    m.dst.req_mem[i] = b;
+    m.dst.req_eph[i] = c;
+    m.dst.nz_cpu[i] = d;
+    m.dst.nz_mem[i] = e;
+    m.dst.num_pods[i] = f;
+  }
+  if (m.begin) {
+    static_assert(sizeof(WinState) % 4 == 0, "WinState by words");
+    for (int32_t i = t0; i < (int32_t)(sizeof(WinState) / 4); i += stride) reinterpret_cast<uint32_t*>(m.win)[i] = 0u;
+    if (blockIdx.x == 0 && threadIdx.x < kLazySlots) m.ring_e[threadIdx.x] = -1;
+  }
+  if (blockIdx.x == 0 && threadIdx.x == 0) {
+    DevState s = *m.st_src;
+    if (m.begin) {
+      s.cursor = m.first;
+      s.end = m.end;
+      s.bcap = 0;
+      if (m.zero_counters) {
+        s.truncations = 0;
+        s.evals = 0;
+        s.scheduled = 0;
+        s.unschedulable = 0;
+        s.batches = 0;
+        s.cuts = 0;
+      }
+      *m.st_dst2 = s;
+      if (m.batches0) *m.batches0 = (unsigned long long)(uint32_t)s.batches;
+    }
+    *m.st_dst = s;
+  }
+}
+
+void launch_lazy_move(const LazyMove& m, hipStream_t stream) {
+  const int blocks = std::min(256, std::max(1, (m.n + 255) / 256));
+  k_lazy_move<<<blocks, 256, 0, stream>>>(m);
+}
+
 __global__ void k_assume(DevCluster c, DevPods P, int32_t pod, int32_t node, int sign) {
   if (threadIdx.x == 0 && blockIdx.x == 0) assume_pod(c, P, P.pods[pod], node, sign);
 }
diff --git a/kube-scheduler-simulator_amd/ksim/engine.py b/kube-scheduler-simulator_amd/ksim/engine.py
--- a/kube-scheduler-simulator_amd/ksim/engine.py
+++ b/kube-scheduler-simulator_amd/ksim/engine.py
@@ -28,7 +28,7 @@
     "ksim_encode_pods", "ksim_encoder_cluster", "ksim_encoder_pods", "ksim_encoder_get_info",
     "ksim_encoder_node_order", "ksim_encoder_string", "ksim_encoder_update_nodes", "ksim_encoder_old_pos",
     "ksim_encoder_bind", "ksim_encoder_unbind", "ksim_encoder_bound_node", "ksim_encoder_changed_rows",
-    "ksim_update_node_rows",
+    "ksim_update_node_rows", "ksim_feed_more_batches",
 ]
 
 
@@ -119,6 +119,9 @@
     L.ksim_time_eval.argtypes = [vp, i32, i32, vp, vp]
     L.ksim_kernel_name.restype = ctypes.c_char_p
     L.ksim_get_diag.argtypes = [vp, vp, i32]
+    if hasattr(L, "ksim_feed_more_batches"):
+        L.ksim_feed_more_batches.argtypes = [i32, i32]
+        L.ksim_feed_more_batches.restype = i32
     L.ksim_batch_geometry.argtypes = [vp, i32]
     L.ksim_set_shard.argtypes = [vp, i32, i32]
     L.ksim_comm_unique_id.argtypes = [vp]
@@ -465,15 +468,17 @@
         self._chk(self.L.ksim_reset_cluster(self.h))
 
     def diag(self) -> dict:
-        out = np.zeros(28, np.int64)
-        n = self.L.ksim_get_diag(self.h, out.ctypes.data_as(ctypes.c_void_p), 28)
+        out = np.zeros(33, np.int64)
+        n = self.L.ksim_get_diag(self.h, out.ctypes.data_as(ctypes.c_void_p), 33)
         if n < 0:
             self._chk(n)
         d = {"batches": int(out[0]), "truncations": int(out[1]), "cuts": int(out[2]),
              "graph_captures": int(out[19]), "dbg": [int(x) for x in out[3:19]], "match_ns": int(out[20]),
              "fw_score_host": int(out[21]), "fw_score_device": int(out[22]), "fw_normalize_cached": int(out[23]),
              "fw_normalize_device": int(out[24]), "variants": int(out[25]), "tb_variant_pods": int(out[26]),
-             "reqtab_runs": int(out[27])}
+             "reqtab_runs": int(out[27]),
+             "feed_syncs": int(out[28]), "feed_past_end": int(out[29]), "feed_fallbacks": int(out[30]),
+             "feed_topups": int(out[31]), "feed_odd_ends": int(out[32])}
         if out[6]:
             d["chain_us"] = {"setup": out[3] / out[6] / 100.0, "rounds": out[4] / out[6] / 100.0,
                              "epilogue": out[5] / out[6] / 100.0, "rounds_per_batch": out[7] / out[6]}
```

Result: faster. 45.57 billion (median of 6 runs) (+3.6%).
